# Black-Phoenix/CUDA-SfM

Measured on NVIDIA B200. Metric: RANSAC hyp*corr evals/s, higher is better.
Workload: dtype f32

## Files before the change

### cuda-sfm_b200/binding.py

```python
from __future__ import annotations

import ctypes as C
import os

HERE = os.path.dirname(os.path.abspath(__file__))


def lib_path() -> str:
    return os.path.join(HERE, "libsfmb200.so")


class SfmError(RuntimeError):
    def __init__(self, code: int, msg: str):
        super().__init__(f"sfmb200 error {code}: {msg}")
        self.code = code


_f = C.POINTER(C.c_float)
_i = C.POINTER(C.c_int32)
_vp = C.c_void_p

SIGNATURES = {
    "sfmb200_last_error": (C.c_char_p, []),
    "sfmb200_version": (C.c_int, []),
    "sfmb200_build_info": (C.c_char_p, []),
    "sfmb200_small_path_debug": (C.c_int, [_vp]),
    "sfmb200_create": (C.c_int, [_f, _f, C.c_int, C.c_int, C.c_int, C.POINTER(_vp)]),
    "sfmb200_destroy": (C.c_int, [_vp]),
    "sfmb200_set_option": (C.c_int, [_vp, C.c_int, C.c_int]),
    "sfmb200_set_stream": (C.c_int, [_vp, _vp]),
    "sfmb200_synchronize": (C.c_int, [_vp]),
    "sfmb200_set_points_sift": (C.c_int, [_vp, _vp, C.c_int]),
    "sfmb200_set_points_sift_filtered": (C.c_int, [_vp, _vp, C.c_int, C.c_float, C.c_float, _vp, C.POINTER(C.c_int32)]),
    "sfmb200_set_points_xy": (C.c_int, [_vp, _vp, C.c_int]),
    "sfmb200_set_points_xy_host": (C.c_int, [_vp, _vp, C.c_int]),
    "sfmb200_set_points_normalised": (C.c_int, [_vp, _vp, C.c_int]),
    "sfmb200_estimate_e": (C.c_int, [_vp, _vp, C.c_int, C.c_uint64, C.c_float]),
    "sfmb200_estimate_e_slice": (C.c_int, [_vp, _vp, C.c_int, C.c_int, C.c_int, C.c_uint64, C.c_float]),
    "sfmb200_copy_to_vbo_coloured": (C.c_int, [_vp, C.c_int, _vp, _vp, C.c_float, C.c_int, C.c_float, C.c_float]),
    "sfmb200_mg_handle_bytes": (C.c_int, []),
    "sfmb200_mg_init": (C.c_int, [_vp, C.c_int, C.c_int, _vp]),
    "sfmb200_mg_connect": (C.c_int, [_vp, _vp]),
    "sfmb200_estimate_e_mg": (C.c_int, [_vp, _vp, C.c_int, C.c_uint64, C.c_float]),
    "sfmb200_mg_status": (C.c_int, [_vp, _vp]),
    "sfmb200_mg_set_timeout_ms": (C.c_int, [_vp, C.c_int]),
    "sfmb200_mg_close": (C.c_int, [_vp]),
    "sfmb200_chain_views": (C.c_int, [_vp, _vp, _vp, _vp, _vp, _vp]),
    "sfmb200_bundle_adjust_global": (C.c_int, [_vp, _vp, _vp, C.c_int, _vp, _vp]),
    "sfmb200_bundle_adjust": (C.c_int, [_vp, C.c_int, C.c_int, _vp]),
    "sfmb200_estimate_e_adaptive": (C.c_int, [_vp, _vp, C.c_int, C.c_int, C.c_int, C.c_uint64, C.c_float, C.c_float, _vp]),
    "sfmb200_best_buffer": (C.c_int, [_vp, C.POINTER(_vp)]),
    "sfmb200_adopt_best": (C.c_int, [_vp, _vp, C.c_int, C.c_uint64]),
    "sfmb200_find_homography": (C.c_int, [_vp, C.c_int, C.c_uint64, C.c_float, _vp, _vp]),
    "sfmb200_refine_e": (C.c_int, [_vp, C.c_int]),
    "sfmb200_get_refit_iterations": (C.c_int, [_vp, _vp]),
    "sfmb200_pose_candidates": (C.c_int, [_vp]),
    "sfmb200_choose_pose": (C.c_int, [_vp]),
    "sfmb200_triangulate": (C.c_int, [_vp]),
    "sfmb200_run_host": (C.c_int, [_vp, _vp, C.c_int, C.c_int, C.c_uint64, C.c_float, _vp, _vp, _vp, _vp, _vp]),
    "sfmb200_run_device": (C.c_int, [_vp, _vp, C.c_int, C.c_int, C.c_uint64, C.c_float]),
    "sfmb200_copy_to_vbo": (C.c_int, [_vp, C.c_int, _vp, _vp]),
    "sfmb200_get_E": (C.c_int, [_vp, _vp]),
    "sfmb200_set_E": (C.c_int, [_vp, _vp]),
    "sfmb200_get_best": (C.c_int, [_vp, _vp, _vp]),
    "sfmb200_get_poses": (C.c_int, [_vp, _vp]),
    "sfmb200_get_pose_index": (C.c_int, [_vp, _vp]),
    "sfmb200_get_points": (C.c_int, [_vp, C.c_int, _vp]),
    "sfmb200_get_points_host": (C.c_int, [_vp, C.c_int, _vp]),
    "sfmb200_get_inlier_counts": (C.c_int, [_vp, C.c_int, _vp]),
    "sfmb200_get_E_candidates": (C.c_int, [_vp, C.c_int, _vp]),
    "sfmb200_get_X": (C.c_int, [_vp, C.c_int, C.c_int, _vp]),
    "sfmb200_get_inlier_mask": (C.c_int, [_vp, C.c_int, _vp]),
    "sfmb200_device_views": (C.c_int, [_vp, C.POINTER(_vp), C.POINTER(_vp), C.POINTER(_vp), C.POINTER(_vp), C.POINTER(C.c_int)]),
    "sfmb200_score_plan": (C.c_int, [_vp, _i]),
    "sfmb200_launch_count": (C.c_int64, [_vp]),
    "sfmb200_stage_times": (C.c_int, [_vp, C.c_int, _vp, C.POINTER(C.c_int)]),
    "sfmb200_fma_probe": (C.c_int, [C.c_int, C.c_int, C.POINTER(C.c_double), C.POINTER(C.c_float)]),
    "sfmb200_host_svd3": (None, [_f, _f, _f, _f]),
    "sfmb200_host_svd3_reference_orientation": (None, [_f, _f, _f, _f]),
    "sfmb200_host_solve_hypothesis": (None, [_f, _f]),
    "sfmb200_host_solve_hypothesis_projector": (None, [_f, _f]),
    "sfmb200_host_null4": (None, [_f, _f]),
    "sfmb200_host_null4_fast": (C.c_int, [_f, _f]),
    "sfmb200_host_dlt_null": (C.c_int, [_f, _f]),
    "sfmb200_host_dlt_null_power4": (None, [_f, _f]),
    "sfmb200_host_inv4": (C.c_int, [_f, _f]),
    "sfmb200_host_sample_indices": (None, [C.c_uint64, C.c_uint64, C.c_int, _i]),
    "sfmb200_host_sample_indices_disjoint": (None, [C.c_uint64, C.c_uint64, C.c_int, _i]),
    "sfmb200_la_mmul": (C.c_int, [_vp, _vp, _vp, C.c_int, C.c_int, C.c_int, _vp]),
    "sfmb200_la_mmul_batched": (C.c_int, [_vp, _vp, _vp, C.c_int, C.c_int, C.c_int, C.c_int, C.c_int, C.c_int, C.c_int, _vp]),
    "sfmb200_la_mmul_transpose_batched": (C.c_int, [_vp, _vp, _vp, C.c_int, C.c_int, C.c_int, C.c_int, C.c_int, C.c_int, C.c_int, _vp]),
    "sfmb200_la_invert": (C.c_int, [_vp, _vp, C.c_int, C.c_int, _vp]),
    "sfmb200_la_svd_batched": (C.c_int, [_vp, _vp, _vp, _vp, C.c_int, C.c_int, C.c_int, _vp]),
    "sfmb200_la_transpose_batched": (C.c_int, [_vp, _vp, C.c_int, C.c_int, C.c_int, _vp]),
    "sfmb200_la_vecnorm": (C.c_int, [_vp, _vp, C.c_int, C.c_int, C.c_float, C.c_float, _vp]),
    "sfmb200_la_elementwise": (C.c_int, [C.c_int, _vp, _vp, C.c_int, _vp]),
    "sfmb200_la_threshold_count": (C.c_int, [_vp, _vp, C.c_int, C.c_int, C.c_float, _vp]),
    "sfmb200_la_row_extraction": (C.c_int, [_vp, _vp, C.c_int, _vp]),
    "sfmb200_la_argmax_first": (C.c_int, [_vp, C.c_int, _i, _vp]),
    "sfmb200_la_copy_point": (C.c_int, [_vp, C.c_int, _vp, _vp, _vp]),
    "sfmb200_la_design_matrix": (C.c_int, [_vp, _vp, _vp, _vp, C.c_int, C.c_int, _vp]),
    "sfmb200_la_normalize_E": (C.c_int, [_vp, C.c_int, _vp]),
    "sfmb200_la_candidate_poses": (C.c_int, [_vp, _vp, _vp, _vp]),
    "sfmb200_la_triangulation_A": (C.c_int, [_vp, _vp, _vp, C.c_int, C.c_int, _vp, _vp, C.c_int, C.c_int, _vp]),
    "sfmb200_la_normalize_pt": (C.c_int, [_vp, _vp, C.c_int, _vp]),
    "sfmb200_la_copy_to_vbo": (C.c_int, [C.c_int, _vp, _vp, C.c_float, _vp]),
}


class Lib:

    def __init__(self, path: str | None = None):
        path = path or lib_path()
        if not os.path.exists(path):
            raise FileNotFoundError(
                f"{path} is missing: build it with `python cuda-sfm_b200/build.py` "
                "(there is no CPU fallback for the sfmb200 hot path)"
            )
        self.path = path
        self.cdll = C.CDLL(path)
        for name, (res, args) in SIGNATURES.items():
            fn = getattr(self.cdll, name)
            fn.restype = res
            fn.argtypes = args
            setattr(self, "_" + name, fn)

    def last_error(self) -> str:
        return self._sfmb200_last_error().decode()

    def call(self, name: str, *args):
        rc = getattr(self, "_" + name)(*args)
        if rc != 0:
            raise SfmError(rc, self.last_error())
        return rc

    def raw(self, name: str):
        return getattr(self, "_" + name)


_LIB: Lib | None = None


def load_library(path: str | None = None) -> Lib:
    global _LIB
    if _LIB is None or (path and path != _LIB.path):
        _LIB = Lib(path)
    return _LIB
```

### cuda-sfm_b200/csrc/api.cu

```cuda
#include <cuda_runtime.h>
#include <math.h>
#include <stdio.h>
#include <string.h>

#include <new>

#include "../../include/sfmb200.h"
#include "internal.cuh"
#include "sampson.cuh"

using namespace sfmb200;

static thread_local char g_err[512] = "";

static int fail(int code, const char* fmt, const char* detail = "") {
    snprintf(g_err, sizeof(g_err), fmt, detail);
    return code;
}
#define CK(call)                                                                     \
    do {                                                                             \
        cudaError_t e_ = (call);                                                     \
        if (e_ != cudaSuccess) return fail(SFMB200_ERR_CUDA, #call ": %s", cudaGetErrorString(e_)); \
    } while (0)
#define CKL()                                                                        \
    do {                                                                             \
        cudaError_t e_ = cudaGetLastError();                                         \
        if (e_ != cudaSuccess) return fail(SFMB200_ERR_CUDA, "kernel launch: %s", cudaGetErrorString(e_)); \
    } while (0)

struct sfmb200_handle {
    DeviceState s;
    RefitState refit;
    BAState ba;
    ChainState chain;
    void* chain_arena;
    GbaState gba;
    void* gba_arena;
    float* gba_stats;
    bool have_chain;
    void* staging_in;
    void* staging_out;
    void* ba_arena;
    MgPeers mg;
    void* mg_local;
    bool mg_connected;
    long long mg_calls;
    int* mg_failed_host;
    int* mg_failed_dev;
    int mg_clock_khz;
    long long mg_timeout_cycles;
    cudaStream_t stream;
    bool own_stream;
    cudaStream_t aux_stream;
    cudaEvent_t ev_fork;
    cudaEvent_t ev_chunk[16];
    int pipeline_chunks;
    int device;
    int sms;
    int compat;
    int score_variant;
    int tri_inliers_only;
    int hyp_solver;
    int small_path;
    long long small_evals;
    int model;
    int H;
    int h_begin;
    float thr;
    bool have_points, have_E, have_candidates, have_pose;
    ScorePlan plan;
    int64_t launches;
    int* filter_scratch;
    float* pack_header;
    float* pack_points;
    float* host_header;
    int* adapt;
    void* arena;
    int profile;
    int prof_cur;
    long long prof_total;
    cudaEvent_t (*prof_ev)[8];
    unsigned char* prof_mask;
};
static const int PROF_RING = 256;
static inline void prof_mark(sfmb200_handle* h, int k) {
    if (!h->profile) return;
    cudaEventRecord(h->prof_ev[h->prof_cur][k], h->stream);
    h->prof_mask[h->prof_cur] |= (unsigned char)(1u << k);
}
static inline void prof_next(sfmb200_handle* h) {
    if (!h->profile) return;
    h->prof_cur = (int)(h->prof_total % PROF_RING);
    h->prof_total++;
    h->prof_mask[h->prof_cur] = 0;
}

struct DeviceScope {
    int prev = -1;
    bool switched = false;
    cudaError_t err = cudaSuccess;
    explicit DeviceScope(const sfmb200_handle* h) {
        if (!h) return;
        err = cudaGetDevice(&prev);
        if (err == cudaSuccess && prev != h->device) {
            err = cudaSetDevice(h->device);
            switched = err == cudaSuccess;
        }
    }
    ~DeviceScope() {
        if (switched) cudaSetDevice(prev);
    }
};
#define ENTER(h)                                                                                          \
    DeviceScope scope_(h);                                                                                \
    if (scope_.err != cudaSuccess) return fail(SFMB200_ERR_CUDA, "cannot make the handle's device current: %s", cudaGetErrorString(scope_.err))

extern "C" {

const char* sfmb200_last_error(void) { return g_err; }
int sfmb200_version(void) { return 100; }

static size_t align_up(size_t v, size_t a) { return (v + a - 1) / a * a; }

int sfmb200_create(const float K[9], const float Kinv[9], int pairs, int max_points, int max_hyp, sfmb200_t** out) {
    if (!K || !Kinv || !out) return fail(SFMB200_ERR_ARG, "null argument%s");
    if (pairs < 1 || max_points < 8 || max_hyp < 1) return fail(SFMB200_ERR_ARG, "pairs >= 1, max_points >= 8, max_hypotheses >= 1 required%s");
    if (pairs > 65535) return fail(SFMB200_ERR_ARG, "at most 65535 pairs per handle (grid.y / grid.z limit)%s");
    int ndev = 0;
    if (cudaGetDeviceCount(&ndev) != cudaSuccess || ndev == 0) {
        cudaGetLastError();
        return fail(SFMB200_ERR_NODEVICE, "no CUDA device: sfmb200 has no CPU fallback%s");
    }
    sfmb200_handle* h = new (std::nothrow) sfmb200_handle();
    if (!h) return fail(SFMB200_ERR_ARG, "out of host memory%s");
    memset(h, 0, sizeof(*h));
    CK(cudaGetDevice(&h->device));
    CK(cudaDeviceGetAttribute(&h->sms, cudaDevAttrMultiProcessorCount, h->device));
    DeviceState& s = h->s;
    s.B = pairs;
    s.n_max = max_points;
    s.h_max = max_hyp;
    s.n = 0;
    s.n_stride = (int)align_up(max_points, SCORE_CHUNK);
    s.h_stride = (int)align_up(max_hyp, 1024);
    s.tiles_max = s.h_stride / SCORE_MIN_TILE;
    memcpy(s.K, K, sizeof(float) * 9);
    memcpy(s.Kinv, Kinv, sizeof(float) * 9);
    size_t B = pairs, off = 0;
    auto carve = [&](size_t bytes) { size_t o = off; off = align_up(off + bytes, 256); return o; };
    size_t o_corr = carve(B * s.n_stride * sizeof(float4));
    size_t o_cs = carve(B * s.n_stride * sizeof(float4));
    size_t o_ec = carve(B * 9 * (size_t)s.h_stride * sizeof(float));
    size_t o_cnt = carve(B * (size_t)s.h_stride * sizeof(int));
    size_t o_td = carve(B * (size_t)s.tiles_max * sizeof(int));
    size_t o_best = carve(B * sizeof(unsigned long long));
    size_t o_E = carve(B * 9 * sizeof(float));
    size_t o_bi = carve(B * sizeof(int));
    size_t o_bc = carve(B * sizeof(int));
    size_t o_P = carve(B * 64 * sizeof(float));
    size_t o_pi = carve(B * sizeof(int));
    size_t o_pts = carve(B * 4 * (size_t)s.n_stride * sizeof(float));
    size_t o_tc = carve(B * sizeof(int));
    size_t o_vote = carve(B * 8 * sizeof(int));
    size_t o_fs = carve(((size_t)max_points / 256 + 2) * sizeof(int));
    size_t o_ph = carve(B * 32 * sizeof(float));
    size_t o_ad = carve(4 * sizeof(int));
    const int refit_blocks = 64;
    size_t o_rc = carve(B * 9 * sizeof(float));
    size_t o_rT = carve(B * 8 * sizeof(float));
    size_t o_rf = carve(B * 4 * sizeof(int));
    size_t o_ri = carve(B * sizeof(int));
    size_t o_rm = carve(B * refit_blocks * 8 * sizeof(float));
    size_t o_rg = carve(B * refit_blocks * 45 * sizeof(float));
    cudaError_t e = cudaMalloc(&h->arena, off);
    if (e != cudaSuccess) {
        delete h;
        return fail(SFMB200_ERR_CUDA, "cudaMalloc(arena): %s", cudaGetErrorString(e));
    }
    char* base = (char*)h->arena;
    s.corr = (float4*)(base + o_corr);
    s.corr_s = (float4*)(base + o_cs);
    s.pt_scale = make_thr_scale(1e-6f).ik;
    s.px = nullptr;
    s.Ecand = (float*)(base + o_ec);
    s.counts = (int*)(base + o_cnt);
    s.tile_done = (int*)(base + o_td);
    s.best = (unsigned long long*)(base + o_best);
    s.E = (float*)(base + o_E);
    s.best_idx = (int*)(base + o_bi);
    s.best_count = (int*)(base + o_bc);
    s.P = (float*)(base + o_P);
    s.P_ind = (int*)(base + o_pi);
    s.points = (float*)(base + o_pts);
    s.tri_count = (int*)(base + o_tc);
    s.vote = (int*)(base + o_vote);
    h->filter_scratch = (int*)(base + o_fs);
    h->pack_header = (float*)(base + o_ph);
    h->pack_points = nullptr;
    h->adapt = (int*)(base + o_ad);
    h->ba.persistent = 1;
    h->refit.cand = (float*)(base + o_rc);
    h->refit.T = (float*)(base + o_rT);
    h->refit.flags = (int*)(base + o_rf);
    h->refit.iters_done = (int*)(base + o_ri);
    h->refit.mom_part = (float*)(base + o_rm);
    h->refit.gram_part = (float*)(base + o_rg);
    h->refit.max_blocks = refit_blocks;
    e = cudaMemset(h->arena, 0, off);
    if (e == cudaSuccess) e = cudaStreamCreateWithFlags(&h->stream, cudaStreamNonBlocking);
    if (e == cudaSuccess) e = cudaMallocHost((void**)&h->host_header, B * 32 * sizeof(float));
    if (e != cudaSuccess) {
        cudaFree(h->arena);
        delete h;
        return fail(SFMB200_ERR_CUDA, "create: %s", cudaGetErrorString(e));
    }
    h->own_stream = true;
    h->compat = 1;
    h->hyp_solver = 1;
    h->score_variant = -1;
    h->tri_inliers_only = 0;
    h->pipeline_chunks = -1;
    h->small_path = -1;
    h->small_evals = 2500000;
    *out = h;
    return SFMB200_OK;
}

int sfmb200_destroy(sfmb200_t* h) {
    ENTER(h);
    if (!h) return SFMB200_OK;
    cudaStreamSynchronize(h->stream);
    sfmb200_mg_close(h);
    if (h->aux_stream) {
        cudaStreamDestroy(h->aux_stream);
        cudaEventDestroy(h->ev_fork);
        for (int i = 0; i < 16; i++) cudaEventDestroy(h->ev_chunk[i]);
    }
    if (h->own_stream) cudaStreamDestroy(h->stream);
    if (h->host_header) cudaFreeHost(h->host_header);
    if (h->prof_ev) {
        for (int i = 0; i < PROF_RING; i++)
            for (int k = 0; k < 8; k++) cudaEventDestroy(h->prof_ev[i][k]);
        delete[] h->prof_ev;
        delete[] h->prof_mask;
    }
    cudaFree(h->arena);
    if (h->chain_arena) cudaFree(h->chain_arena);
    if (h->gba_arena) cudaFree(h->gba_arena);
    if (h->ba_arena) cudaFree(h->ba_arena);
    if (h->staging_in) cudaFree(h->staging_in);
    if (h->staging_out) cudaFree(h->staging_out);
    delete h;
    return SFMB200_OK;
}

int sfmb200_set_option(sfmb200_t* h, int option, int value) {
    ENTER(h);
    if (!h) return fail(SFMB200_ERR_ARG, "null handle%s");
    switch (option) {
        case SFMB200_OPT_COMPAT: h->compat = value ? 1 : 0; break;
        case SFMB200_OPT_SCORE_VARIANT:
            if (value < -1 || value >= score_num_variants()) return fail(SFMB200_ERR_ARG, "score variant out of range%s");
            h->score_variant = value;
            break;
        case SFMB200_OPT_TRI_INLIERS_ONLY: h->tri_inliers_only = value ? 1 : 0; break;
        case SFMB200_OPT_HYP_SOLVER:
            if (value < 0 || value > 1) return fail(SFMB200_ERR_ARG, "hypothesis solver must be 0 (Jacobi) or 1 (Cholesky projector)%s");
            h->hyp_solver = value;
            break;
        case SFMB200_OPT_BA_PERSISTENT: h->ba.persistent = value ? 1 : 0; break;
        case SFMB200_OPT_BATCH_PIPELINE:
            if (value < -1 || value > 16) return fail(SFMB200_ERR_ARG, "batch pipeline chunks must be -1 (auto), 0 / 1 (off) or 2..16%s");
            h->pipeline_chunks = value;
            break;
        case SFMB200_OPT_SAMPLER:
            if (value < 0 || value > 1) return fail(SFMB200_ERR_ARG, "sampler must be 0 (independent subsets) or 1 (disjoint permutation)%s");
            h->s.sampler = value;
            break;
        case SFMB200_OPT_SCORE_METRIC:
            if (value < 0 || value > 1) return fail(SFMB200_ERR_ARG, "score metric must be 0 (Sampson error) or 1 (symmetric epipolar distance)%s");
            h->s.metric = value;
            break;
        case SFMB200_OPT_SMALL_PATH:
            if (value < -1 || value > 1) return fail(SFMB200_ERR_ARG, "small path must be -1 (auto), 0 (never) or 1 (whenever eligible)%s");
            h->small_path = value;
            break;
        case SFMB200_OPT_SMALL_PATH_EVALS:
            if (value < 0) return fail(SFMB200_ERR_ARG, "evaluation limit must be >= 0%s");
            h->small_evals = value;
            break;
        case SFMB200_OPT_PROFILE:
            if (value && !h->prof_ev) {
                h->prof_ev = new cudaEvent_t[PROF_RING][8];
                h->prof_mask = new unsigned char[PROF_RING]();
                for (int i = 0; i < PROF_RING; i++)
                    for (int k = 0; k < 8; k++) CK(cudaEventCreate(&h->prof_ev[i][k]));
            }
            h->profile = value ? 1 : 0;
            h->prof_total = 0;
            h->prof_cur = 0;
            if (h->prof_mask) memset(h->prof_mask, 0, PROF_RING);
            break;
        default: return fail(SFMB200_ERR_ARG, "unknown option%s");
    }
    return SFMB200_OK;
}

int sfmb200_set_stream(sfmb200_t* h, void* stream) {
    ENTER(h);
    if (!h) return fail(SFMB200_ERR_ARG, "null handle%s");
    if (h->own_stream) {
        cudaStreamSynchronize(h->stream);
        cudaStreamDestroy(h->stream);
        h->own_stream = false;
    }
    h->stream = (cudaStream_t)stream;
    return SFMB200_OK;
}

int sfmb200_synchronize(sfmb200_t* h) {
    ENTER(h);
    if (!h) return fail(SFMB200_ERR_ARG, "null handle%s");
    CK(cudaStreamSynchronize(h->stream));
    return SFMB200_OK;
}

static int check_n(sfmb200_t* h, const void* p, int n) {
    if (!h || !p) return fail(SFMB200_ERR_ARG, "null argument%s");
    if (n < 8 || n > h->s.n_max) return fail(SFMB200_ERR_ARG, "n must be in [8, max_points]%s");
    return SFMB200_OK;
}

int sfmb200_set_points_sift(sfmb200_t* h, const void* d_sift, int n) {
    ENTER(h);
    int rc = check_n(h, d_sift, n);
    if (rc) return rc;
    if (h->s.B != 1) return fail(SFMB200_ERR_ARG, "SiftPoint ingest needs pairs == 1%s");
    h->s.n = n;
    launch_ingest_sift(h->s, d_sift, n, h->stream);
    CKL();
    h->launches++;
    h->have_points = true;
    h->have_chain = false;
    return SFMB200_OK;
}
int sfmb200_set_points_sift_filtered(sfmb200_t* h, const void* d_sift, int n, float min_score, float max_ambiguity,
                                     int32_t* d_kept_index, int32_t* h_kept) {
    ENTER(h);
    int rc = check_n(h, d_sift, n);
    if (rc) return rc;
    if (h->s.B != 1) return fail(SFMB200_ERR_ARG, "SiftPoint ingest needs pairs == 1%s");
    h->have_points = false;
    launch_ingest_sift_filtered(h->s, d_sift, n, min_score, max_ambiguity, h->filter_scratch, d_kept_index, h->stream);
    CKL();
    h->launches += 3;
    int kept = 0;
    int blocks = (n + 255) / 256;
    CK(cudaMemcpyAsync(&kept, h->filter_scratch + blocks, sizeof(int), cudaMemcpyDeviceToHost, h->stream));
    CK(cudaStreamSynchronize(h->stream));
    if (h_kept) *h_kept = kept;
    if (kept < 8) return fail(SFMB200_ERR_STATE, "fewer than 8 correspondences survive the match filter%s");
    h->s.n = kept;
    h->have_points = true;
    h->have_chain = false;
    return SFMB200_OK;
}
static int ingest_xy(sfmb200_t* h, const float* d_px, int n, float scale) {
    int rc = check_n(h, d_px, n);
    if (rc) return rc;
    h->s.n = n;
    if (scale > 0.0f) h->s.pt_scale = scale;
    prof_mark(h, 0);
    launch_ingest_xy(h->s, d_px, n, h->stream);
    prof_mark(h, 1);
    CKL();
    h->launches++;
    h->have_points = true;
    h->have_chain = false;
    return SFMB200_OK;
}
int sfmb200_set_points_xy(sfmb200_t* h, const float* d_px, int n) {
    ENTER(h);
    return ingest_xy(h, d_px, n, 0.0f);
}
static int ensure_staging(sfmb200_handle* h, bool in, bool out) {
    if (in && !h->staging_in) {
        CK(cudaMalloc(&h->staging_in, (size_t)h->s.B * h->s.n_stride * 4 * sizeof(float)));
        h->s.px = (float*)h->staging_in;
    }
    if (out && !h->staging_out) {
        CK(cudaMalloc(&h->staging_out, (size_t)h->s.B * 4 * (size_t)h->s.n_max * sizeof(float)));
        h->pack_points = (float*)h->staging_out;
    }
    return SFMB200_OK;
}

static int ingest_xy_host(sfmb200_t* h, const float* h_px, int n, float scale) {
    int rc = check_n(h, h_px, n);
    if (rc) return rc;
    if ((rc = ensure_staging(h, true, false))) return rc;
    CK(cudaMemcpyAsync(h->s.px, h_px, (size_t)h->s.B * n * 4 * sizeof(float), cudaMemcpyHostToDevice, h->stream));
    return ingest_xy(h, h->s.px, n, scale);
}
int sfmb200_set_points_xy_host(sfmb200_t* h, const float* h_px, int n) {
    ENTER(h);
    return ingest_xy_host(h, h_px, n, 0.0f);
}
int sfmb200_set_points_normalised(sfmb200_t* h, const float* d_x, int n) {
    ENTER(h);
    int rc = check_n(h, d_x, n);
    if (rc) return rc;
    h->s.n = n;
    launch_ingest_normalised(h->s, d_x, n, h->stream);
    CKL();
    h->launches++;
    h->have_points = true;
    h->have_chain = false;
    return SFMB200_OK;
}

static int ensure_scaled(sfmb200_handle* h, float scale) {
    if (h->s.pt_scale == scale) return SFMB200_OK;
    h->s.pt_scale = scale;
    launch_rescale_points(h->s, h->stream);
    CKL();
    h->launches++;
    return SFMB200_OK;
}

static void score_essential(sfmb200_handle* h, const DeviceState& s, int H, int h_offset, float thr) {
    if (s.metric == 0) launch_score(s, h->plan, H, h_offset, thr, h->stream);
    else launch_score_symmetric(s, h->plan, H, h_offset, thr, h->stream);
}
static ScorePlan plan_essential(const sfmb200_handle* h, int n, int H) {
    return h->s.metric == 0 ? make_score_plan(h->s.B, n, H, h->score_variant, h->sms) : make_score_plan_homography(h->s.B, n, H, h->sms);
}

constexpr int SMALL_PATH_MAX_PAIRS = 4;
static bool small_path_ok(const sfmb200_handle* h, int H, bool pose) {
    if (h->small_path == 0 || h->profile || h->hyp_solver != 1 || h->s.skip != nullptr || h->s.metric != 0) return false;
    if (h->score_variant >= 0 && h->small_path != 1) return false;
    if (pose && !h->compat) return false;
    if (H > small_path_max_hypotheses()) return false;
    if (h->small_path == 1) return true;
    if (h->s.B > SMALL_PATH_MAX_PAIRS) return false;
    return (long long)h->s.n * (long long)H <= h->small_evals;
}

int sfmb200_estimate_e_slice(sfmb200_t* h, const int32_t* d_idx, int H_total, int h_begin, int H, uint64_t seed,
                             float thr) {
    ENTER(h);
    if (!h) return fail(SFMB200_ERR_ARG, "null handle%s");
    if (!h->have_points) return fail(SFMB200_ERR_STATE, "estimate_e before set_points%s");
    if (H < 1 || H > h->s.h_max || h_begin < 0 || (long long)h_begin + H > (long long)H_total)
        return fail(SFMB200_ERR_ARG, "hypothesis slice out of range / above max_hypotheses%s");
    if (!(thr > 0.0f)) return fail(SFMB200_ERR_ARG, "threshold must be positive%s");
    if (!d_idx && h->s.sampler == 1 && 8ll * H_total > (long long)h->s.n)
        return fail(SFMB200_ERR_ARG, "the disjoint-permutation sampler needs 8 * H_total <= n (the reference uses H = N / 8)%s");
    h->H = H;
    h->h_begin = h_begin;
    h->thr = thr;
    if (int rc = ensure_scaled(h, make_thr_scale(thr).ik)) return rc;
    if (small_path_ok(h, H, false)) {
        CK(launch_small_path(h->s, nullptr, d_idx, (long long)H_total * 8, H, h_begin, seed, thr, h->compat, 0, SMALL_ESTIMATE, h->stream));
        memset(&h->plan, 0, sizeof(h->plan));
        h->plan.variant = -2;
        h->launches += 1;
    } else {
        h->plan = plan_essential(h, h->s.n, H);
        launch_hypgen(h->s, d_idx, (long long)H_total * 8, H, h_begin, seed, h->hyp_solver, h->stream);
        prof_mark(h, 2);
        CKL();
        score_essential(h, h->s, H, h_begin, thr);
        prof_mark(h, 3);
        CKL();
        launch_select(h->s, h_begin, h->stream);
        prof_mark(h, 4);
        CKL();
        h->launches += 3;
    }
    h->have_candidates = true;
    h->have_E = true;
    h->have_pose = false;
    h->have_chain = false;
    h->model = 0;
    return SFMB200_OK;
}

int sfmb200_find_homography(sfmb200_t* h, int loops, uint64_t seed, float thresh, float* h_H, int32_t* h_matches) {
    ENTER(h);
    if (!h) return fail(SFMB200_ERR_ARG, "null handle%s");
    if (!h->have_points) return fail(SFMB200_ERR_STATE, "find_homography before set_points%s");
    if (loops < 1 || loops > h->s.h_max) return fail(SFMB200_ERR_ARG, "loops out of range / above max_hypotheses%s");
    if (!(thresh > 0.0f)) return fail(SFMB200_ERR_ARG, "threshold must be positive%s");
    const float* Kc = h->s.K;
    const float f = Kc[0];
    const bool isotropic = f > 0.0f && fabsf(Kc[4] - f) <= 1e-6f * f && Kc[1] == 0.0f && Kc[3] == 0.0f && Kc[6] == 0.0f &&
                           Kc[7] == 0.0f && Kc[8] == 1.0f;
    if (!isotropic)
        return fail(SFMB200_ERR_ARG, "find_homography needs K = [f 0 cx; 0 f cy; 0 0 1] (square pixels, no skew): the pixel threshold is applied as thresh / f%s");
    const float thresh_n = thresh / f;
    const float thr2 = thresh_n * thresh_n;
    if (int rc = ensure_scaled(h, 1.0f)) return rc;
    h->H = loops;
    h->h_begin = 0;
    h->thr = thr2;
    h->plan = make_score_plan_homography(h->s.B, h->s.n, loops, h->sms);
    launch_hypgen(h->s, nullptr, (long long)loops * 8, loops, 0, seed, 2, h->stream);
    CKL();
    launch_score_homography(h->s, h->plan, loops, 0, thr2, h->stream);
    CKL();
    launch_select(h->s, 0, h->stream);
    CKL();
    h->launches += 3;
    h->have_candidates = true;
    h->have_E = false;
    h->have_pose = false;
    h->have_chain = false;
    h->model = 1;
    if (h_H) CK(cudaMemcpyAsync(h_H, h->s.E, (size_t)h->s.B * 9 * sizeof(float), cudaMemcpyDeviceToHost, h->stream));
    if (h_matches) CK(cudaMemcpyAsync(h_matches, h->s.best_count, (size_t)h->s.B * sizeof(int), cudaMemcpyDeviceToHost, h->stream));
    if (h_H || h_matches) CK(cudaStreamSynchronize(h->stream));
    if (h_H) {
        for (int b = 0; b < h->s.B; b++) {
            float* Hm = h_H + 9 * b;
            double T[9], R[9];
            for (int i = 0; i < 3; i++)
                for (int j = 0; j < 3; j++) {
                    double a = 0.0;
                    for (int k = 0; k < 3; k++) a += (double)Hm[3 * i + k] * (double)h->s.Kinv[3 * k + j];
                    T[3 * i + j] = a;
                }
            for (int i = 0; i < 3; i++)
                for (int j = 0; j < 3; j++) {
                    double a = 0.0;
                    for (int k = 0; k < 3; k++) a += (double)h->s.K[3 * i + k] * T[3 * k + j];
                    R[3 * i + j] = a;
                }
            const double inv = fabs(R[8]) > 1e-12 ? 1.0 / R[8] : 1.0;
            for (int i = 0; i < 9; i++) Hm[i] = (float)(R[i] * inv);
        }
    }
    return SFMB200_OK;
}
int sfmb200_estimate_e(sfmb200_t* h, const int32_t* d_idx, int H, uint64_t seed, float thr) {
    ENTER(h);
    return sfmb200_estimate_e_slice(h, d_idx, H, 0, H, seed, thr);
}

int sfmb200_estimate_e_adaptive(sfmb200_t* h, const int32_t* d_idx, int H_max, int first_round, int growth,
                                uint64_t seed, float thr, float confidence, int32_t* h_used) {
    ENTER(h);
    if (!h) return fail(SFMB200_ERR_ARG, "null handle%s");
    if (!h->have_points) return fail(SFMB200_ERR_STATE, "estimate_e before set_points%s");
    if (H_max < 1 || first_round < 1 || growth < 2) return fail(SFMB200_ERR_ARG, "H_max >= 1, first_round >= 1, growth >= 2 required%s");
    if (!(thr > 0.0f)) return fail(SFMB200_ERR_ARG, "threshold must be positive%s");
    if (!(confidence > 0.0f && confidence < 1.0f)) return fail(SFMB200_ERR_ARG, "confidence must be in (0, 1)%s");
    {
        long long lo = 0, hi = first_round;
        while (lo < H_max) {
            if (hi > H_max) hi = H_max;
            if (hi - lo > h->s.h_max) return fail(SFMB200_ERR_ARG, "a round exceeds max_hypotheses of the handle%s");
            lo = hi;
            hi *= growth;
        }
    }
    const double log1mp = log1p(-(double)confidence);
    if (int rc = ensure_scaled(h, make_thr_scale(thr).ik)) return rc;
    CK(cudaMemsetAsync(h->adapt, 0, 4 * sizeof(int), h->stream));
    DeviceState s = h->s;
    s.skip = h->adapt;
    long long lo = 0, hi = first_round;
    int rounds = 0;
    while (lo < H_max) {
        if (hi > H_max) hi = H_max;
        const int Hr = (int)(hi - lo);
        h->plan = plan_essential(h, s.n, Hr);
        launch_hypgen(s, d_idx, (long long)H_max * 8, Hr, (int)lo, seed, h->hyp_solver, h->stream, rounds > 0);
        CKL();
        score_essential(h, s, Hr, (int)lo, thr);
        CKL();
        launch_adaptive_decide(s, h->adapt, (int)lo, (int)hi, log1mp, hi >= H_max, h->stream);
        CKL();
        h->launches += 3;
        rounds++;
        h->H = Hr;
        h->h_begin = (int)lo;
        lo = hi;
        hi *= growth;
    }
    h->thr = thr;
    h->have_candidates = false;
    h->have_E = true;
    h->have_pose = false;
    h->have_chain = false;
    h->model = 0;
    if (h_used) {
        CK(cudaMemcpyAsync(h_used, h->adapt + 1, sizeof(int), cudaMemcpyDeviceToHost, h->stream));
        CK(cudaStreamSynchronize(h->stream));
    }
    return SFMB200_OK;
}

struct MgBlob {
    cudaIpcMemHandle_t ipc;
    unsigned char uuid[16];
};
int sfmb200_mg_handle_bytes(void) { return (int)sizeof(MgBlob); }

int sfmb200_mg_init(sfmb200_t* h, int rank, int world, void* h_handle_out) {
    ENTER(h);
    if (!h || !h_handle_out) return fail(SFMB200_ERR_ARG, "null argument%s");
    if (world < 1 || world > MG_MAX_WORLD || rank < 0 || rank >= world) return fail(SFMB200_ERR_ARG, "bad rank / world (at most 16 ranks)%s");
    if (h->mg_local) return fail(SFMB200_ERR_STATE, "mg_init called twice%s");
    const size_t bytes = mg_buffer_bytes(h->s.B, world);
    CK(cudaMalloc(&h->mg_local, bytes));
    CK(cudaMemset(h->mg_local, 0, bytes));
    CK(cudaHostAlloc((void**)&h->mg_failed_host, sizeof(int), cudaHostAllocMapped));
    *h->mg_failed_host = 0;
    CK(cudaHostGetDevicePointer((void**)&h->mg_failed_dev, h->mg_failed_host, 0));
    MgBlob blob;
    memset(&blob, 0, sizeof(blob));
    CK(cudaIpcGetMemHandle(&blob.ipc, h->mg_local));
    cudaDeviceProp prop;
    CK(cudaGetDeviceProperties(&prop, h->device));
    memcpy(blob.uuid, prop.uuid.bytes, 16);
    memcpy(h_handle_out, &blob, sizeof(blob));
    memset(&h->mg, 0, sizeof(h->mg));
    h->mg.rank = rank;
    h->mg.world = world;
    h->mg.base[rank] = (unsigned long long*)h->mg_local;
    h->mg_connected = false;
    h->mg_calls = 0;
    int clock_khz = 0;
    cudaDeviceGetAttribute(&clock_khz, cudaDevAttrClockRate, h->device);
    h->mg_clock_khz = clock_khz > 0 ? clock_khz : 1900000;
    h->mg_timeout_cycles = 2000LL * h->mg_clock_khz;
    return SFMB200_OK;
}

int sfmb200_mg_set_timeout_ms(sfmb200_t* h, int ms) {
    ENTER(h);
    if (!h || ms < 1) return fail(SFMB200_ERR_ARG, "timeout must be >= 1 ms%s");
    if (!h->mg_local) return fail(SFMB200_ERR_STATE, "mg_set_timeout_ms before mg_init%s");
    h->mg_timeout_cycles = (long long)ms * h->mg_clock_khz;
    return SFMB200_OK;
}

int sfmb200_mg_connect(sfmb200_t* h, const void* h_handles) {
    ENTER(h);
    if (!h || !h_handles) return fail(SFMB200_ERR_ARG, "null argument%s");
    if (!h->mg_local) return fail(SFMB200_ERR_STATE, "mg_connect before mg_init%s");
    if (h->mg_connected) return fail(SFMB200_ERR_STATE, "mg_connect called twice%s");
    const MgBlob* all = (const MgBlob*)h_handles;
    int ndev = 0;
    CK(cudaGetDeviceCount(&ndev));
    for (int r = 0; r < h->mg.world; r++) {
        if (r == h->mg.rank) continue;
        int peer_dev = -1;
        for (int d = 0; d < ndev && peer_dev < 0; d++) {
            cudaDeviceProp prop;
            CK(cudaGetDeviceProperties(&prop, d));
            if (memcmp(prop.uuid.bytes, all[r].uuid, 16) == 0) peer_dev = d;
        }
        if (peer_dev < 0) return fail(SFMB200_ERR_ARG, "mg_connect: a peer's device is not visible to this process%s");
        if (peer_dev != h->device) {
            int native = 0;
            CK(cudaDeviceGetP2PAttribute(&native, cudaDevP2PAttrNativeAtomicSupported, h->device, peer_dev));
            if (!native) return fail(SFMB200_ERR_STATE, "mg_connect: no native P2P atomics between this device and a peer (not NVLink-connected)%s");
        }
        void* p = nullptr;
        CK(cudaIpcOpenMemHandle(&p, all[r].ipc, cudaIpcMemLazyEnablePeerAccess));
        h->mg.base[r] = (unsigned long long*)p;
    }
    h->mg_connected = true;
    return SFMB200_OK;
}

int sfmb200_mg_close(sfmb200_t* h) {
    ENTER(h);
    if (!h) return SFMB200_OK;
    if (h->mg_local) {
        cudaStreamSynchronize(h->stream);
        for (int r = 0; r < h->mg.world; r++)
            if (r != h->mg.rank && h->mg.base[r]) cudaIpcCloseMemHandle(h->mg.base[r]);
        cudaFree(h->mg_local);
        cudaFreeHost(h->mg_failed_host);
        h->mg_local = nullptr;
        h->mg_failed_host = nullptr;
        h->mg_failed_dev = nullptr;
        h->mg_connected = false;
        memset(&h->mg, 0, sizeof(h->mg));
    }
    return SFMB200_OK;
}

int sfmb200_estimate_e_mg(sfmb200_t* h, const int32_t* d_idx, int H_total, uint64_t seed, float thr) {
    ENTER(h);
    if (!h) return fail(SFMB200_ERR_ARG, "null handle%s");
    if (!h->mg_connected) return fail(SFMB200_ERR_STATE, "estimate_e_mg before mg_init / mg_connect%s");
    if (*(volatile int*)h->mg_failed_host != 0) {
        h->have_E = false;
        h->have_candidates = false;
        return fail(SFMB200_ERR_STATE, "the peer exchange timed out earlier (a rank is lost or late): sfmb200_mg_close + mg_init + mg_connect on every rank%s");
    }
    const int world = h->mg.world, rank = h->mg.rank;
    if (H_total < world) return fail(SFMB200_ERR_ARG, "fewer hypotheses than ranks%s");
    const long long base = H_total / world, rem = H_total % world;
    const long long lo = rank * base + (rank < rem ? rank : rem), cnt = base + (rank < rem ? 1 : 0);
    int rc = sfmb200_estimate_e_slice(h, d_idx, H_total, (int)lo, (int)cnt, seed, thr);
    if (rc) return rc;
    launch_mg_exchange(h->s, h->mg, h->mg_calls, H_total, h->mg_timeout_cycles, h->mg_failed_dev, h->stream);
    CKL();
    h->mg_calls++;
    h->launches += 2;
    h->have_candidates = false;
    return SFMB200_OK;
}

int sfmb200_mg_status(sfmb200_t* h, int32_t* h_timeouts) {
    ENTER(h);
    if (!h || !h_timeouts) return fail(SFMB200_ERR_ARG, "null argument%s");
    *h_timeouts = 0;
    if (!h->mg_failed_host) return SFMB200_OK;
    CK(cudaStreamSynchronize(h->stream));
    *h_timeouts = *(volatile int*)h->mg_failed_host;
    if (*h_timeouts != 0) h->have_E = false;
    return SFMB200_OK;
}

int sfmb200_best_buffer(sfmb200_t* h, uint64_t** d_best) {
    ENTER(h);
    if (!h || !d_best) return fail(SFMB200_ERR_ARG, "null argument%s");
    *d_best = (uint64_t*)h->s.best;
    return SFMB200_OK;
}
int sfmb200_adopt_best(sfmb200_t* h, const int32_t* d_idx, int H_total, uint64_t seed) {
    ENTER(h);
    if (!h) return fail(SFMB200_ERR_ARG, "null handle%s");
    if (!h->have_points) return fail(SFMB200_ERR_STATE, "adopt_best before set_points%s");
    if (h->model != 0 || !(h->thr > 0.0f))
        return fail(SFMB200_ERR_STATE, "adopt_best follows an essential-matrix estimate (estimate_e / estimate_e_slice) on this handle%s");
    launch_regen_best(h->s, d_idx, (long long)H_total * 8, seed, h->hyp_solver, h->stream);
    CKL();
    h->launches++;
    h->have_E = true;
    h->have_pose = false;
    h->have_chain = false;
    h->model = 0;
    return SFMB200_OK;
}

int sfmb200_refine_e(sfmb200_t* h, int iterations) {
    ENTER(h);
    if (!h) return fail(SFMB200_ERR_ARG, "null handle%s");
    if (iterations < 0 || iterations > 64) return fail(SFMB200_ERR_ARG, "iterations must be in [0, 64]%s");
    if (!h->have_E || !h->have_points) return fail(SFMB200_ERR_STATE, "refine_e before an essential matrix exists%s");
    if (iterations == 0) return SFMB200_OK;
    h->launches += launch_refit(h->s, h->refit, h->thr > 0 ? h->thr : 1e-6f, iterations, h->stream);
    CKL();
    h->have_pose = false;
    h->have_chain = false;
    return SFMB200_OK;
}
static int ensure_ba_arena(sfmb200_handle* h) {
    if (h->ba_arena) return SFMB200_OK;
    const DeviceState& s = h->s;
    const size_t B = s.B;
    int ba_blocks = (592 + s.B - 1) / s.B;
    ba_blocks = ba_blocks < 2 ? 2 : (ba_blocks > 296 ? 296 : ba_blocks);
    size_t off = 0;
    auto carve = [&](size_t bytes) { size_t o = off; off = align_up(off + bytes, 256); return o; };
    size_t o_bp = carve(B * 2 * 3 * (size_t)s.n_stride * sizeof(float));
    size_t o_ba = carve(B * (size_t)s.n_stride);
    size_t o_bc2 = carve(B * 24 * sizeof(float));
    size_t o_bd = carve(B * 6 * sizeof(double));
    size_t o_bi2 = carve(B * 8 * sizeof(int));
    size_t o_bf = carve(B * 8 * sizeof(float));
    size_t o_bpart = carve(B * ba_blocks * 34 * sizeof(double));
    size_t o_bpart2 = carve(B * ba_blocks * 2 * sizeof(double));
    size_t o_bs = carve(B * 8 * sizeof(float));
    size_t o_bcand = carve(B * 32 * sizeof(float));
    size_t o_bbase = carve(B * sizeof(int));
    CK(cudaMalloc(&h->ba_arena, off));
    CK(cudaMemsetAsync(h->ba_arena, 0, off, h->stream));
    char* base = (char*)h->ba_arena;
    h->ba.pts = (float*)(base + o_bp);
    h->ba.active = (unsigned char*)(base + o_ba);
    h->ba.cam = (float*)(base + o_bc2);
    h->ba.dc = (double*)(base + o_bd);
    h->ba.ctl_i = (int*)(base + o_bi2);
    h->ba.ctl_f = (float*)(base + o_bf);
    h->ba.part = (double*)(base + o_bpart);
    h->ba.part2 = (double*)(base + o_bpart2);
    h->ba.stats = (float*)(base + o_bs);
    h->ba.cand = (float*)(base + o_bcand);
    h->ba.base_count = (int*)(base + o_bbase);
    h->ba.max_blocks = ba_blocks;
    return SFMB200_OK;
}

int sfmb200_bundle_adjust(sfmb200_t* h, int outer_rounds, int iterations, float* h_stats) {
    ENTER(h);
    if (!h) return fail(SFMB200_ERR_ARG, "null handle%s");
    if (outer_rounds < 1 || outer_rounds > 64 || iterations < 1 || iterations > 256)
        return fail(SFMB200_ERR_ARG, "outer_rounds in [1, 64] and iterations in [1, 256] required%s");
    if (!h->have_points || !h->have_E || !h->have_pose || h->model != 0)
        return fail(SFMB200_ERR_STATE, "bundle_adjust needs an essential matrix and a chosen pose%s");
    const float thr = h->thr > 0 ? h->thr : 1e-6f;
    if (int rc = ensure_ba_arena(h)) return rc;
    for (int r = 0; r < outer_rounds; r++) {
        h->launches += launch_bundle_adjust(h->s, h->ba, thr, iterations, 1e-3f, h->tri_inliers_only, r == 0, h->ba.stats, h->stream);
        CKL();
    }
    if (h_stats) {
        CK(cudaMemcpyAsync(h_stats, h->ba.stats, (size_t)h->s.B * 8 * sizeof(float), cudaMemcpyDeviceToHost, h->stream));
        CK(cudaStreamSynchronize(h->stream));
    }
    return SFMB200_OK;
}

int sfmb200_chain_views(sfmb200_t* h, float* d_cloud, int32_t* d_count, float* h_cameras, float* h_scales, int32_t* h_used) {
    ENTER(h);
    if (!h) return fail(SFMB200_ERR_ARG, "null handle%s");
    if (h->s.B > 256) return fail(SFMB200_ERR_ARG, "chain_views handles at most 256 pairs (257 views)%s");
    if (!h->have_points || !h->have_E || !h->have_pose || h->model != 0)
        return fail(SFMB200_ERR_STATE, "chain_views needs an essential matrix, a chosen pose and triangulated points per pair%s");
    const size_t B = h->s.B;
    if (!h->chain_arena) {
        size_t off = 0;
        auto carve = [&](size_t bytes) { size_t o = off; off = align_up(off + bytes, 256); return o; };
        size_t o_h = carve(B * 2048 * sizeof(int)), o_m = carve(B * sizeof(int)), o_u = carve(B * sizeof(int));
        size_t o_s = carve(B * sizeof(unsigned long long)), o_c = carve(B * sizeof(int)), o_sc = carve(B * sizeof(float));
        size_t o_cs = carve(B * sizeof(float)), o_cam = carve((B + 1) * 12 * sizeof(float));
        CK(cudaMalloc(&h->chain_arena, off));
        char* base = (char*)h->chain_arena;
        h->chain.hist = (int*)(base + o_h);
        h->chain.median_bin = (int*)(base + o_m);
        h->chain.used = (int*)(base + o_u);
        h->chain.bin_sum = (unsigned long long*)(base + o_s);
        h->chain.bin_cnt = (int*)(base + o_c);
        h->chain.scales = (float*)(base + o_sc);
        h->chain.cum_scales = (float*)(base + o_cs);
        h->chain.cameras = (float*)(base + o_cam);
        CK(cudaMemsetAsync(h->chain_arena, 0, off, h->stream));
    }
    h->launches += launch_chain(h->s, h->chain, h->thr > 0 ? h->thr : 1e-6f, d_cloud, d_count, h->stream);
    CKL();
    if (h_cameras) CK(cudaMemcpyAsync(h_cameras, h->chain.cameras, (B + 1) * 12 * sizeof(float), cudaMemcpyDeviceToHost, h->stream));
    if (h_scales) CK(cudaMemcpyAsync(h_scales, h->chain.scales, B * sizeof(float), cudaMemcpyDeviceToHost, h->stream));
    if (h_used) CK(cudaMemcpyAsync(h_used, h->chain.used, B * sizeof(int), cudaMemcpyDeviceToHost, h->stream));
    if (h_cameras || h_scales || h_used) CK(cudaStreamSynchronize(h->stream));
    h->have_chain = true;
    return SFMB200_OK;
}

int sfmb200_bundle_adjust_global(sfmb200_t* h, float* d_cloud, const int32_t* d_count, int iterations, float* h_cameras,
                                 float* h_stats) {
    ENTER(h);
    if (!h || !d_cloud || !d_count) return fail(SFMB200_ERR_ARG, "null argument%s");
    if (iterations < 1 || iterations > 1000) return fail(SFMB200_ERR_ARG, "iterations must be in [1, 1000]%s");
    if (h->s.B > GBA_MAX_PAIRS) return fail(SFMB200_ERR_ARG, "bundle_adjust_global handles at most 16 pairs (17 views)%s");
    if (!h->have_chain || !h->chain_arena || !h->have_points || !h->have_E || !h->have_pose || h->model != 0)
        return fail(SFMB200_ERR_STATE, "bundle_adjust_global follows chain_views (cloud and count from that call)%s");
    const DeviceState& s = h->s;
    if (!h->gba_arena) {
        const size_t V = s.B + 1, n = s.n_max;
        const int nb = 148;
        size_t off = 0;
        auto carve = [&](size_t bytes) { size_t o = off; off = align_up(off + bytes, 256); return o; };
        size_t o_cam = carve(2 * V * 12 * sizeof(float)), o_pts = carve(2 * 3 * n * sizeof(float)), o_obs = carve(n * sizeof(unsigned int));
        size_t o_lin = carve(n * 9 * sizeof(float)), o_part = carve(gba_part_doubles(s.B, nb) * sizeof(double));
        size_t o_p2 = carve((size_t)nb * 2 * sizeof(double)), o_dc = carve(6 * (size_t)s.B * sizeof(double));
        size_t o_ci = carve(8 * sizeof(int)), o_cf = carve(8 * sizeof(float)), o_st = carve(8 * sizeof(float));
        CK(cudaMalloc(&h->gba_arena, off));
        CK(cudaMemsetAsync(h->gba_arena, 0, off, h->stream));
        char* base = (char*)h->gba_arena;
        h->gba.cam = (float*)(base + o_cam);
        h->gba.pts = (float*)(base + o_pts);
        h->gba.obs = (unsigned int*)(base + o_obs);
        h->gba.lin = (float*)(base + o_lin);
        h->gba.part = (double*)(base + o_part);
        h->gba.part2 = (double*)(base + o_p2);
        h->gba.dc = (double*)(base + o_dc);
        h->gba.ctl_i = (int*)(base + o_ci);
        h->gba.ctl_f = (float*)(base + o_cf);
        h->gba.nb = nb;
        h->gba_stats = (float*)(base + o_st);
    }
    float* d_stats = h->gba_stats;
    h->launches += launch_global_ba(h->s, h->chain, h->gba, h->thr > 0 ? h->thr : 1e-6f, iterations, d_cloud, d_count, d_stats, h->stream);
    CKL();
    const size_t B = h->s.B;
    if (h_cameras) CK(cudaMemcpyAsync(h_cameras, h->chain.cameras, (B + 1) * 12 * sizeof(float), cudaMemcpyDeviceToHost, h->stream));
    if (h_stats) CK(cudaMemcpyAsync(h_stats, d_stats, 8 * sizeof(float), cudaMemcpyDeviceToHost, h->stream));
    if (h_cameras || h_stats) CK(cudaStreamSynchronize(h->stream));
    return SFMB200_OK;
}

int sfmb200_get_refit_iterations(sfmb200_t* h, int32_t* h_iters) {
    ENTER(h);
    if (!h || !h_iters) return fail(SFMB200_ERR_ARG, "null argument%s");
    CK(cudaMemcpyAsync(h_iters, h->refit.iters_done, (size_t)h->s.B * sizeof(int), cudaMemcpyDeviceToHost, h->stream));
    CK(cudaStreamSynchronize(h->stream));
    return SFMB200_OK;
}

int sfmb200_pose_candidates(sfmb200_t* h) {
    ENTER(h);
    if (!h) return fail(SFMB200_ERR_ARG, "null handle%s");
    if (!h->have_E) return fail(SFMB200_ERR_STATE, "pose_candidates before an essential matrix exists%s");
    launch_pose_candidates(h->s, h->compat, h->stream);
    prof_mark(h, 5);
    CKL();
    h->launches++;
    h->have_pose = true;
    return SFMB200_OK;
}
int sfmb200_choose_pose(sfmb200_t* h) {
    ENTER(h);
    if (!h) return fail(SFMB200_ERR_ARG, "null handle%s");
    if (!h->have_pose || !h->have_points) return fail(SFMB200_ERR_STATE, "choose_pose before pose_candidates%s");
    launch_choose_pose(h->s, h->compat, h->thr > 0 ? h->thr : 1e-6f, h->stream);
    prof_mark(h, 6);
    CKL();
    h->launches++;
    return SFMB200_OK;
}
int sfmb200_triangulate(sfmb200_t* h) {
    ENTER(h);
    if (!h) return fail(SFMB200_ERR_ARG, "null handle%s");
    if (!h->have_pose || !h->have_points) return fail(SFMB200_ERR_STATE, "triangulate before pose_candidates%s");
    launch_triangulate(h->s, h->tri_inliers_only, h->thr > 0 ? h->thr : 1e-6f, h->stream);
    prof_mark(h, 7);
    CKL();
    h->launches++;
    return SFMB200_OK;
}

static int run_stages(sfmb200_t* h, int H, uint64_t seed, float thr) {
    if (!h->have_points) return fail(SFMB200_ERR_STATE, "run before set_points%s");
    if (H < 1 || H > h->s.h_max) return fail(SFMB200_ERR_ARG, "H out of range / above max_hypotheses%s");
    if (!(thr > 0.0f)) return fail(SFMB200_ERR_ARG, "threshold must be positive%s");
    h->H = H;
    h->h_begin = 0;
    h->thr = thr;
    if (int rc = ensure_scaled(h, make_thr_scale(thr).ik)) return rc;
    h->plan = plan_essential(h, h->s.n, H);
    int chunks = h->pipeline_chunks;
    if (chunks < 0) chunks = 1;
    if (chunks > h->s.B) chunks = h->s.B;
    if (chunks >= 2) {
        if (!h->aux_stream) {
            CK(cudaStreamCreateWithFlags(&h->aux_stream, cudaStreamNonBlocking));
            CK(cudaEventCreateWithFlags(&h->ev_fork, cudaEventDisableTiming));
            for (int i = 0; i < 16; i++) CK(cudaEventCreateWithFlags(&h->ev_chunk[i], cudaEventDisableTiming));
        }
        CK(cudaEventRecord(h->ev_fork, h->stream));
        CK(cudaStreamWaitEvent(h->aux_stream, h->ev_fork, 0));
        const int per = (h->s.B + chunks - 1) / chunks;
        int used = 0;
        for (int c = 0, b0 = 0; b0 < h->s.B; c++, b0 += per, used++) {
            const DeviceState v = sub_batch(h->s, b0, b0 + per <= h->s.B ? per : h->s.B - b0);
            launch_hypgen(v, nullptr, (long long)H * 8, H, 0, seed, h->hyp_solver, h->aux_stream);
            CKL();
            CK(cudaEventRecord(h->ev_chunk[c], h->aux_stream));
        }
        for (int c = 0, b0 = 0; b0 < h->s.B; c++, b0 += per) {
            const DeviceState v = sub_batch(h->s, b0, b0 + per <= h->s.B ? per : h->s.B - b0);
            CK(cudaStreamWaitEvent(h->stream, h->ev_chunk[c], 0));
            ScorePlan keep = h->plan;
            h->plan = h->s.metric == 0 ? make_score_plan(v.B, v.n, H, h->score_variant, h->sms) : make_score_plan_homography(v.B, v.n, H, h->sms);
            score_essential(h, v, H, 0, thr);
            CKL();
            h->plan = keep;
        }
        h->launches += 2 * used - 2;
    } else {
        launch_hypgen(h->s, nullptr, (long long)H * 8, H, 0, seed, h->hyp_solver, h->stream);
        prof_mark(h, 2);
        CKL();
        score_essential(h, h->s, H, 0, thr);
        prof_mark(h, 3);
        CKL();
    }
    launch_select_pose_choose(h->s, 0, h->compat, h->stream);
    prof_mark(h, 4);
    prof_mark(h, 5);
    CKL();
    h->launches += 3;
    if (!h->compat) {
        launch_choose_pose(h->s, 0, thr, h->stream);
        CKL();
        h->launches++;
    }
    prof_mark(h, 6);
    h->have_candidates = h->have_E = h->have_pose = true;
    h->have_chain = false;
    h->model = 0;
    return sfmb200_triangulate(h);
}

static int run_small(sfmb200_t* h, const float* d_px, int n, int H, uint64_t seed, float thr) {
    if (!d_px || n < 8 || n > h->s.n_max || H < 1 || H > h->s.h_max) return 0;
    const int n_before = h->s.n;
    h->s.n = n;
    const bool ok = small_path_ok(h, H, true);
    h->s.n = n_before;
    if (!ok) return 0;
    h->s.n = n;
    h->s.pt_scale = make_thr_scale(thr).ik;
    cudaError_t e = launch_small_path(h->s, d_px, nullptr, (long long)H * 8, H, 0, seed, thr, h->compat, h->tri_inliers_only,
                                      SMALL_INGEST | SMALL_ESTIMATE | SMALL_POSE | SMALL_TRI, h->stream);
    if (e != cudaSuccess) return fail(SFMB200_ERR_CUDA, "fused small-problem launch: %s", cudaGetErrorString(e));
    h->H = H;
    h->h_begin = 0;
    h->thr = thr;
    h->model = 0;
    memset(&h->plan, 0, sizeof(h->plan));
    h->plan.variant = -2;
    h->launches += 1;
    h->have_points = h->have_candidates = h->have_E = h->have_pose = true;
    h->have_chain = false;
    return 1;
}

int sfmb200_run_device(sfmb200_t* h, const float* d_px, int n, int H, uint64_t seed, float thr) {
    ENTER(h);
    if (!h) return fail(SFMB200_ERR_ARG, "null handle%s");
    if (!(thr > 0.0f)) return fail(SFMB200_ERR_ARG, "threshold must be positive%s");
    prof_next(h);
    if (int rc = run_small(h, d_px, n, H, seed, thr)) return rc < 0 ? rc : SFMB200_OK;
    int rc = ingest_xy(h, d_px, n, make_thr_scale(thr).ik);
    if (rc) return rc;
    return run_stages(h, H, seed, thr);
}

__global__ void pack_results_kernel(DeviceState s, float* header, float* points, int want_points) {
    const int b = blockIdx.y;
    if (blockIdx.x == 0 && threadIdx.x < 32) {
        const int t = threadIdx.x;
        float v = 0.0f;
        if (t < 9) v = s.E[(size_t)b * 9 + t];
        else if (t < 25) v = s.P[(size_t)b * 64 + 16 * s.P_ind[b] + (t - 9)];
        else if (t == 25) v = __int_as_float(s.P_ind[b]);
        else if (t == 26) v = __int_as_float(s.best_count[b]);
        else if (t == 27) v = __int_as_float(s.best_idx[b]);
        header[(size_t)b * 32 + t] = v;
    }
    if (!want_points) return;
    const int i = blockIdx.x * blockDim.x + threadIdx.x;
    if (i >= s.n) return;
    const float* in = s.points + (size_t)b * 4 * s.n_stride;
    float* out = points + (size_t)b * 4 * s.n;
#pragma unroll
    for (int r = 0; r < 4; r++) out[(size_t)r * s.n + i] = in[(size_t)r * s.n_stride + i];
}

static void* pinned_alias(const void* host) {
    if (!host) return nullptr;
    cudaPointerAttributes a;
    if (cudaPointerGetAttributes(&a, host) != cudaSuccess) {
        cudaGetLastError();
        return nullptr;
    }
    return a.type == cudaMemoryTypeHost ? a.devicePointer : nullptr;
}

int sfmb200_run_host(sfmb200_t* h, const float* h_px, int n, int H, uint64_t seed, float thr, float* h_E, float* h_P,
                     int32_t* h_pose_index, int32_t* h_inliers, float* h_points) {
    ENTER(h);
    if (!h) return fail(SFMB200_ERR_ARG, "null handle%s");
    if (!(thr > 0.0f)) return fail(SFMB200_ERR_ARG, "threshold must be positive%s");
    prof_next(h);
    const float scale = make_thr_scale(thr).ik;
    const size_t zero_copy_limit = 4u << 20;
    const size_t in_bytes = (size_t)h->s.B * (size_t)(n > 0 ? n : 0) * 4 * sizeof(float);
    const float* px_alias = in_bytes <= zero_copy_limit ? (const float*)pinned_alias(h_px) : nullptr;
    int rc = 0;
    const bool small_shape = h_px && n >= 8 && n <= h->s.n_max && H >= 1 && H <= h->s.h_max;
    if (px_alias) {
        rc = run_small(h, px_alias, n, H, seed, thr);
    } else if (small_shape) {
        if ((rc = ensure_staging(h, true, false))) return rc;
        CK(cudaMemcpyAsync(h->s.px, h_px, (size_t)h->s.B * n * 4 * sizeof(float), cudaMemcpyHostToDevice, h->stream));
        rc = run_small(h, h->s.px, n, H, seed, thr);
        if (rc == 0) {
            if ((rc = ingest_xy(h, h->s.px, n, scale))) return rc;
            if ((rc = run_stages(h, H, seed, thr))) return rc;
            rc = 1;
        }
    }
    if (rc < 0) return rc;
    if (rc == 0) {
        rc = px_alias ? ingest_xy(h, px_alias, n, scale) : ingest_xy_host(h, h_px, n, scale);
        if (rc) return rc;
        if ((rc = run_stages(h, H, seed, thr))) return rc;
    }
    DeviceState& s = h->s;
    const size_t B = s.B;
    float* pts_alias = B * 4 * (size_t)s.n * sizeof(float) <= zero_copy_limit ? (float*)pinned_alias(h_points) : nullptr;
    if (h_points && !pts_alias && (rc = ensure_staging(h, false, true))) return rc;
    dim3 grid(h_points ? (s.n + 255) / 256 : 1, (unsigned)B);
    pack_results_kernel<<<grid, 256, 0, h->stream>>>(s, h->host_header, pts_alias ? pts_alias : h->pack_points, h_points ? 1 : 0);
    CKL();
    h->launches++;
    if (h_points && !pts_alias)
        CK(cudaMemcpyAsync(h_points, h->pack_points, B * 4 * (size_t)s.n * sizeof(float), cudaMemcpyDeviceToHost, h->stream));
    CK(cudaStreamSynchronize(h->stream));
    for (size_t b = 0; b < B; b++) {
        const float* hd = h->host_header + b * 32;
        if (h_E) memcpy(h_E + b * 9, hd, 9 * sizeof(float));
        if (h_P) memcpy(h_P + b * 16, hd + 9, 16 * sizeof(float));
        if (h_pose_index) memcpy(h_pose_index + b, hd + 25, sizeof(int32_t));
        if (h_inliers) memcpy(h_inliers + b, hd + 26, sizeof(int32_t));
    }
    return SFMB200_OK;
}

int sfmb200_copy_to_vbo(sfmb200_t* h, int pair, float* d_pos, float* d_col) {
    ENTER(h);
    if (!h || pair < 0 || pair >= h->s.B) return fail(SFMB200_ERR_ARG, "bad handle / pair%s");
    launch_vbo(h->s, pair, d_pos, d_col, 1.0f, h->stream);
    CKL();
    h->launches++;
    CK(cudaStreamSynchronize(h->stream));
    return SFMB200_OK;
}

int sfmb200_copy_to_vbo_coloured(sfmb200_t* h, int pair, float* d_pos, float* d_col, float scale, int mode, float z_near, float z_far) {
    ENTER(h);
    if (!h || pair < 0 || pair >= h->s.B) return fail(SFMB200_ERR_ARG, "bad handle / pair%s");
    if (mode < 0 || mode > 2) return fail(SFMB200_ERR_ARG, "colour mode must be 0 (ones), 1 (inlier / outlier) or 2 (depth ramp)%s");
    if (mode == 1 && (!h->have_E || h->model != 0)) return fail(SFMB200_ERR_STATE, "inlier colouring needs an essential matrix%s");
    launch_vbo_colour(h->s, pair, d_pos, d_col, scale, mode, h->thr > 0 ? h->thr : 1e-6f, z_near, z_far, h->stream);
    CKL();
    h->launches++;
    CK(cudaStreamSynchronize(h->stream));
    return SFMB200_OK;
}

int sfmb200_get_E(sfmb200_t* h, float* h_E) {
    ENTER(h);
    if (!h || !h_E) return fail(SFMB200_ERR_ARG, "null argument%s");
    CK(cudaMemcpyAsync(h_E, h->s.E, (size_t)h->s.B * 9 * sizeof(float), cudaMemcpyDeviceToHost, h->stream));
    CK(cudaStreamSynchronize(h->stream));
    return SFMB200_OK;
}
int sfmb200_set_E(sfmb200_t* h, const float* h_E) {
    ENTER(h);
    if (!h || !h_E) return fail(SFMB200_ERR_ARG, "null argument%s");
    CK(cudaMemcpyAsync(h->s.E, h_E, (size_t)h->s.B * 9 * sizeof(float), cudaMemcpyHostToDevice, h->stream));
    CK(cudaStreamSynchronize(h->stream));
    h->have_E = true;
    h->have_pose = false;
    h->have_chain = false;
    h->model = 0;
    if (!(h->thr > 0)) h->thr = 1e-6f;
    return SFMB200_OK;
}
int sfmb200_get_best(sfmb200_t* h, int32_t* h_index, int32_t* h_count) {
    ENTER(h);
    if (!h) return fail(SFMB200_ERR_ARG, "null argument%s");
    if (h_index) CK(cudaMemcpyAsync(h_index, h->s.best_idx, (size_t)h->s.B * sizeof(int), cudaMemcpyDeviceToHost, h->stream));
    if (h_count) CK(cudaMemcpyAsync(h_count, h->s.best_count, (size_t)h->s.B * sizeof(int), cudaMemcpyDeviceToHost, h->stream));
    CK(cudaStreamSynchronize(h->stream));
    return SFMB200_OK;
}
int sfmb200_get_poses(sfmb200_t* h, float* h_P) {
    ENTER(h);
    if (!h || !h_P) return fail(SFMB200_ERR_ARG, "null argument%s");
    CK(cudaMemcpyAsync(h_P, h->s.P, (size_t)h->s.B * 64 * sizeof(float), cudaMemcpyDeviceToHost, h->stream));
    CK(cudaStreamSynchronize(h->stream));
    return SFMB200_OK;
}
int sfmb200_get_pose_index(sfmb200_t* h, int32_t* h_ind) {
    ENTER(h);
    if (!h || !h_ind) return fail(SFMB200_ERR_ARG, "null argument%s");
    CK(cudaMemcpyAsync(h_ind, h->s.P_ind, (size_t)h->s.B * sizeof(int), cudaMemcpyDeviceToHost, h->stream));
    CK(cudaStreamSynchronize(h->stream));
    return SFMB200_OK;
}
static int check_pair(sfmb200_t* h, int pair, const void* p) {
    if (!h || !p) return fail(SFMB200_ERR_ARG, "null argument%s");
    if (pair < 0 || pair >= h->s.B) return fail(SFMB200_ERR_ARG, "pair out of range%s");
    return SFMB200_OK;
}
int sfmb200_get_points(sfmb200_t* h, int pair, float* d_points) {
    ENTER(h);
    int rc = check_pair(h, pair, d_points);
    if (rc) return rc;
    const DeviceState& s = h->s;
    CK(cudaMemcpy2DAsync(d_points, (size_t)s.n * sizeof(float), s.points + (size_t)pair * 4 * s.n_stride,
                         (size_t)s.n_stride * sizeof(float), (size_t)s.n * sizeof(float), 4, cudaMemcpyDeviceToDevice,
                         h->stream));
    return SFMB200_OK;
}
int sfmb200_get_points_host(sfmb200_t* h, int pair, float* h_points) {
    ENTER(h);
    int rc = check_pair(h, pair, h_points);
    if (rc) return rc;
    const DeviceState& s = h->s;
    CK(cudaMemcpy2DAsync(h_points, (size_t)s.n * sizeof(float), s.points + (size_t)pair * 4 * s.n_stride,
                         (size_t)s.n_stride * sizeof(float), (size_t)s.n * sizeof(float), 4, cudaMemcpyDeviceToHost,
                         h->stream));
    CK(cudaStreamSynchronize(h->stream));
    return SFMB200_OK;
}
int sfmb200_get_inlier_counts(sfmb200_t* h, int pair, int32_t* d_counts) {
    ENTER(h);
    int rc = check_pair(h, pair, d_counts);
    if (rc) return rc;
    if (!h->have_candidates) return fail(SFMB200_ERR_STATE, "no estimate yet%s");
    CK(cudaMemcpyAsync(d_counts, h->s.counts + (size_t)pair * h->s.h_stride, (size_t)h->H * sizeof(int),
                       cudaMemcpyDeviceToDevice, h->stream));
    return SFMB200_OK;
}
int sfmb200_get_E_candidates(sfmb200_t* h, int pair, float* d_E) {
    ENTER(h);
    int rc = check_pair(h, pair, d_E);
    if (rc) return rc;
    if (!h->have_candidates) return fail(SFMB200_ERR_STATE, "no estimate yet%s");
    launch_export_ecand(h->s, pair, h->H, d_E, h->stream);
    CKL();
    h->launches++;
    return SFMB200_OK;
}
int sfmb200_get_X(sfmb200_t* h, int pair, int image, float* d_X) {
    ENTER(h);
    int rc = check_pair(h, pair, d_X);
    if (rc) return rc;
    if (image < 0 || image > 1) return fail(SFMB200_ERR_ARG, "image must be 0 or 1%s");
    if (!h->have_points) return fail(SFMB200_ERR_STATE, "no points yet%s");
    launch_export_X(h->s, pair, image, d_X, h->stream);
    CKL();
    h->launches++;
    return SFMB200_OK;
}
int sfmb200_get_inlier_mask(sfmb200_t* h, int pair, uint8_t* d_mask) {
    ENTER(h);
    int rc = check_pair(h, pair, d_mask);
    if (rc) return rc;
    if (!(h->have_E || h->model == 1) || !h->have_points) return fail(SFMB200_ERR_STATE, "no model yet%s");
    launch_inlier_mask(h->s, pair, h->thr > 0 ? h->thr : 1e-6f, h->model, d_mask, h->stream);
    CKL();
    h->launches++;
    return SFMB200_OK;
}
int sfmb200_device_views(sfmb200_t* h, float** d_E, float** d_P, int32_t** d_pose_index, float** d_points,
                         int* point_stride) {
    ENTER(h);
    if (!h) return fail(SFMB200_ERR_ARG, "null handle%s");
    if (d_E) *d_E = h->s.E;
    if (d_P) *d_P = h->s.P;
    if (d_pose_index) *d_pose_index = h->s.P_ind;
    if (d_points) *d_points = h->s.points;
    if (point_stride) *point_stride = h->s.n_stride;
    return SFMB200_OK;
}
int sfmb200_score_plan(sfmb200_t* h, int32_t out[4]) {
    ENTER(h);
    if (!h || !out) return fail(SFMB200_ERR_ARG, "null argument%s");
    out[0] = h->plan.variant;
    out[1] = h->plan.tiles;
    out[2] = h->plan.ctas;
    out[3] = h->plan.hyp_per_cta;
    return SFMB200_OK;
}
int64_t sfmb200_launch_count(sfmb200_t* h) { return h ? h->launches : 0; }

int sfmb200_stage_times(sfmb200_t* h, int max_sets, float* ms, int* sets) {
    ENTER(h);
    if (!h || !ms || !sets) return fail(SFMB200_ERR_ARG, "null argument%s");
    *sets = 0;
    if (!h->prof_ev) return fail(SFMB200_ERR_STATE, "profiling was never enabled%s");
    CK(cudaStreamSynchronize(h->stream));
    long long have = h->prof_total < PROF_RING ? h->prof_total : PROF_RING;
    long long first = h->prof_total - have;
    for (long long t = first; t < h->prof_total && *sets < max_sets; t++) {
        int i = (int)(t % PROF_RING);
        if (h->prof_mask[i] != 0xFF) continue;
        for (int k = 0; k < 7; k++) CK(cudaEventElapsedTime(&ms[(size_t)(*sets) * 7 + k], h->prof_ev[i][k], h->prof_ev[i][k + 1]));
        (*sets)++;
    }
    return SFMB200_OK;
}

int sfmb200_small_path_debug(int64_t* d_stamps) {
    small_path_set_debug((long long*)d_stamps);
    return SFMB200_OK;
}

int sfmb200_fma_probe(int mode, int iters, double* fmas, float* ms) {
    if (!fmas || !ms || iters < 1 || mode < 0 || mode > 4) return fail(SFMB200_ERR_ARG, "bad argument%s");
    float* sink = nullptr;
    cudaEvent_t e0, e1;
    CK(cudaMalloc(&sink, 256));
    CK(cudaEventCreate(&e0));
    CK(cudaEventCreate(&e1));
    launch_fma_probe(mode, 4, 0, sink);
    CK(cudaEventRecord(e0, 0));
    *fmas = launch_fma_probe(mode, iters, 0, sink);
    CK(cudaEventRecord(e1, 0));
    CK(cudaEventSynchronize(e1));
    CKL();
    CK(cudaEventElapsedTime(ms, e0, e1));
    cudaEventDestroy(e0);
    cudaEventDestroy(e1);
    cudaFree(sink);
    return SFMB200_OK;
}

}
```

### cuda-sfm_b200/csrc/internal.cuh

```cuda
#pragma once
#include <cuda_runtime.h>
#include <stdint.h>

namespace sfmb200 {

struct ScorePlan {
    int variant;
    int hyp_per_cta;
    int tiles;
    int n_units;
    long long total_units;
    int ctas;
};

#ifndef SFMB200_SCORE_CHUNK
#define SFMB200_SCORE_CHUNK 512
#endif
constexpr int SCORE_CHUNK = SFMB200_SCORE_CHUNK;
constexpr int SCORE_GRAIN = 64;
constexpr int SCORE_MIN_TILE = 256;

struct DeviceState {
    int B;
    int pair0;
    int n_max;
    int h_max;
    int n;
    int n_stride;
    int h_stride;
    int tiles_max;
    float Kinv[9];
    float K[9];

    float pt_scale;
    float4* corr;
    float4* corr_s;
    float* px;
    float* Ecand;
    int* counts;
    int* tile_done;
    unsigned long long* best;
    float* E;
    int* best_idx;
    int* best_count;
    float* P;
    int* P_ind;
    float* points;
    int* tri_count;
    int* vote;
    int sampler;
    int metric;
    const int* skip;
};

inline DeviceState sub_batch(const DeviceState& s, int b0, int nb) {
    DeviceState v = s;
    const size_t b = (size_t)b0;
    v.B = nb;
    v.pair0 = s.pair0 + b0;
    v.corr += b * s.n_stride;
    v.corr_s += b * s.n_stride;
    v.Ecand += b * 9 * s.h_stride;
    v.counts += b * s.h_stride;
    v.tile_done += b * s.tiles_max;
    v.best += b;
    v.E += b * 9;
    v.best_idx += b;
    v.best_count += b;
    v.P += b * 64;
    v.P_ind += b;
    v.points += b * 4 * s.n_stride;
    v.tri_count += b;
    v.vote += b * 8;
    return v;
}

struct RefitState {
    float* cand;
    float* T;
    int* flags;
    int* iters_done;
    float* mom_part;
    float* gram_part;
    int max_blocks;
};
int launch_refit(const DeviceState& s, const RefitState& r, float thr, int iterations, cudaStream_t st);

struct BAState {
    float* pts;
    unsigned char* active;
    float* cam;
    double* dc;
    int* ctl_i;
    float* ctl_f;
    double* part;
    double* part2;
    int persistent;
    float* stats;
    int* base_count;
    float* cand;
    int max_blocks;
};
constexpr int MG_MAX_WORLD = 16;
struct MgPeers {
    unsigned long long* base[MG_MAX_WORLD];
    int rank, world;
};
void launch_mg_exchange(const DeviceState& s, const MgPeers& peers, long long call, int H_total, long long timeout_cycles,
                        int* d_failed, cudaStream_t st);
size_t mg_buffer_bytes(int B, int world);

struct ChainState {
    int* hist;
    int* median_bin;
    int* used;
    unsigned long long* bin_sum;
    int* bin_cnt;
    float* scales;
    float* cum_scales;
    float* cameras;
};
int launch_chain(const DeviceState& s, const ChainState& c, float thr, float* d_cloud, int* d_count, cudaStream_t st);

struct GbaState {
    float* cam;
    float* pts;
    unsigned int* obs;
    float* lin;
    double* part;
    double* part2;
    double* dc;
    int* ctl_i;
    float* ctl_f;
    int nb;
};
constexpr int GBA_MAX_PAIRS = 16;
size_t gba_part_doubles(int pairs, int nb);
int launch_global_ba(const DeviceState& s, const ChainState& c, const GbaState& g, float thr, int iterations, float* d_cloud,
                     const int* d_count, float* d_stats, cudaStream_t st);

int launch_bundle_adjust(const DeviceState& s, const BAState& ba, float thr, int iterations, float lambda0,
                         int tri_inliers_only, int first_round, float* d_stats, cudaStream_t st);

void launch_ingest_sift(const DeviceState& s, const void* d_sift, int n, cudaStream_t st);
void launch_ingest_sift_filtered(const DeviceState& s, const void* d_sift, int n, float min_score, float max_ambiguity,
                                 int* d_scratch, int* d_kept_index, cudaStream_t st);
void launch_ingest_xy(const DeviceState& s, const float* d_px, int n, cudaStream_t st);
void launch_ingest_normalised(const DeviceState& s, const float* d_x, int n, cudaStream_t st);
void launch_rescale_points(const DeviceState& s, cudaStream_t st);
void launch_hypgen(const DeviceState& s, const int32_t* d_idx, long long idx_pair_stride, int H, int h_offset,
                   unsigned long long seed, int solver, cudaStream_t st, int keep_best = 0);
void launch_adaptive_decide(const DeviceState& s, int* d_adapt, int round_begin, int done_after, double log1mp, int last,
                            cudaStream_t st);
ScorePlan make_score_plan(int B, int n, int H, int variant_override, int sms);
int score_num_variants();
void launch_score(const DeviceState& s, const ScorePlan& plan, int H, int h_offset, float thr, cudaStream_t st);
void launch_score_homography(const DeviceState& s, ScorePlan& plan, int H, int h_offset, float thr2, cudaStream_t st);
void launch_score_symmetric(const DeviceState& s, ScorePlan& plan, int H, int h_offset, float thr, cudaStream_t st);
ScorePlan make_score_plan_homography(int B, int n, int H, int sms);
void launch_select(const DeviceState& s, int h_offset, cudaStream_t st);
void launch_regen_best(const DeviceState& s, const int32_t* d_idx, long long idx_pair_stride,
                       unsigned long long seed, int solver, cudaStream_t st);
void launch_pose_candidates(const DeviceState& s, int compat, cudaStream_t st);
void launch_select_pose_choose(const DeviceState& s, int h_offset, int compat, cudaStream_t st);
void launch_choose_pose(const DeviceState& s, int compat, float thr, cudaStream_t st);
void launch_triangulate(const DeviceState& s, int inliers_only, float thr, cudaStream_t st);
void launch_vbo(const DeviceState& s, int pair, float* d_pos, float* d_col, float scale, cudaStream_t st);
void launch_vbo_colour(const DeviceState& s, int pair, float* d_pos, float* d_col, float scale, int mode, float thr, float z_near,
                       float z_far, cudaStream_t st);
void launch_export_ecand(const DeviceState& s, int pair, int H, float* d_out_Hx9, cudaStream_t st);
void launch_export_X(const DeviceState& s, int pair, int image, float* d_out_3xN, cudaStream_t st);
void launch_inlier_mask(const DeviceState& s, int pair, float thr, int model, unsigned char* d_mask, cudaStream_t st);

enum { SMALL_INGEST = 1, SMALL_ESTIMATE = 2, SMALL_POSE = 4, SMALL_TRI = 8 };
int small_path_max_hypotheses();
void small_path_set_debug(long long* d_stamps);
cudaError_t launch_small_path(const DeviceState& s, const float* d_px, const int32_t* d_idx, long long idx_pair_stride, int H,
                              int h_offset, unsigned long long seed, float thr, int compat, int inliers_only, int mask,
                              cudaStream_t st);

#ifdef SFMB200_PDL
__device__ __forceinline__ void pdl_wait() { asm volatile("griddepcontrol.wait;" ::: "memory"); }
__device__ __forceinline__ void pdl_trigger() { asm volatile("griddepcontrol.launch_dependents;" ::: "memory"); }
template <typename... KArgs, typename... Args>
inline void launch_dep(void (*kernel)(KArgs...), dim3 grid, dim3 block, size_t smem, cudaStream_t st, Args... args) {
    cudaLaunchConfig_t cfg = {};
    cfg.gridDim = grid;
    cfg.blockDim = block;
    cfg.dynamicSmemBytes = smem;
    cfg.stream = st;
    cudaLaunchAttribute attr[1];
    attr[0].id = cudaLaunchAttributeProgrammaticStreamSerialization;
    attr[0].val.programmaticStreamSerializationAllowed = 1;
    cfg.attrs = attr;
    cfg.numAttrs = 1;
    cudaLaunchKernelEx(&cfg, kernel, KArgs(args)...);
}
#else
__device__ __forceinline__ void pdl_wait() {}
__device__ __forceinline__ void pdl_trigger() {}
template <typename... KArgs, typename... Args>
inline void launch_dep(void (*kernel)(KArgs...), dim3 grid, dim3 block, size_t smem, cudaStream_t st, Args... args) {
    kernel<<<grid, block, smem, st>>>(KArgs(args)...);
}
#endif

double launch_fma_probe(int mode, int iters, cudaStream_t st, float* d_sink);

}
```

### cuda-sfm_b200/csrc/score.cu

```cuda
#include <math.h>

#include <mutex>

#include "internal.cuh"
#include "sampson.cuh"

#ifndef SFMB200_SCORE_UNROLL
#define SFMB200_SCORE_UNROLL 2
#endif

namespace sfmb200 {

constexpr int kScoreUnroll = SFMB200_SCORE_UNROLL;

__device__ __forceinline__ uint32_t smem_u32(const void* p) { return (uint32_t)__cvta_generic_to_shared(p); }

__device__ __forceinline__ void mbar_init(uint64_t* bar, int count) {
    asm volatile("mbarrier.init.shared::cta.b64 [%0], %1;" ::"r"(smem_u32(bar)), "r"(count));
}
__device__ __forceinline__ void mbar_expect_tx(uint64_t* bar, uint32_t bytes) {
    asm volatile("mbarrier.arrive.expect_tx.shared::cta.b64 _, [%0], %1;" ::"r"(smem_u32(bar)), "r"(bytes) : "memory");
}
__device__ __forceinline__ void mbar_wait(uint64_t* bar, uint32_t parity) {
    uint32_t done;
    do {
        asm volatile(
            "{\n"
            ".reg .pred p;\n"
            "mbarrier.try_wait.parity.shared::cta.b64 p, [%1], %2;\n"
            "selp.u32 %0, 1, 0, p;\n"
            "}\n"
            : "=r"(done)
            : "r"(smem_u32(bar)), "r"(parity)
            : "memory");
    } while (!done);
}
__device__ __forceinline__ void tma_load_1d(void* dst, const void* src, uint32_t bytes, uint64_t* bar) {
    asm volatile("cp.async.bulk.shared::cluster.global.mbarrier::complete_tx::bytes [%0], [%1], %2, [%3];" ::"r"(
                     smem_u32(dst)),
                 "l"(src), "r"(bytes), "r"(smem_u32(bar))
                 : "memory");
}

__device__ __forceinline__ unsigned long long warp_max_u64(unsigned long long v) {
#pragma unroll
    for (int o = 16; o > 0; o >>= 1) {
        unsigned long long w = __shfl_xor_sync(0xFFFFFFFFu, v, o);
        v = w > v ? w : v;
    }
    return v;
}

struct ChunkWalk {
    long long u, end;
    int n_units, n, T;
    int b, t, p0, cnt;
    int seg_p0, seg_pts;
    int left;
    bool seg_first, seg_last;
    __device__ __forceinline__ void init(long long u0, long long u1, int n_units_, int n_, int T_) {
        u = u0; end = u1; n_units = n_units_; n = n_; T = T_;
        left = 0; cnt = 0; p0 = 0;
    }
    __device__ __forceinline__ bool next() {
        if (left == 0) {
            if (u >= end) return false;
            long long bt = u / n_units;
            int pu = (int)(u - bt * n_units);
            long long seg_units = end - u;
            if (seg_units > n_units - pu) seg_units = n_units - pu;
            b = (int)(bt / T);
            t = (int)(bt - (long long)b * T);
            seg_p0 = pu * SCORE_GRAIN;
            int p1 = (pu + (int)seg_units) * SCORE_GRAIN;
            if (p1 > n) p1 = n;
            seg_pts = p1 - seg_p0;
            left = seg_pts;
            u += seg_units;
            p0 = seg_p0;
            seg_first = true;
        } else {
            p0 += cnt;
            seg_first = false;
        }
        cnt = left < SCORE_CHUNK ? left : SCORE_CHUNK;
        left -= cnt;
        seg_last = (left == 0);
        return true;
    }
};

template <int HPT, int THREADS>
__device__ __forceinline__ void segment_epilogue(const DeviceState& s, int b, int t, int H, int h_offset,
                                                 const unsigned int* cnt, bool full, int inc, int total,
                                                 unsigned long long* red, int* s_last) {
    constexpr int HPC = HPT * THREADS;
    const int tid = threadIdx.x;
    int* counts = s.counts + (size_t)b * s.h_stride;
    unsigned long long key = 0ull;
    bool do_argmax;
    if (full) {
#pragma unroll
        for (int j = 0; j < HPT; j++) {
            int h = t * HPC + j * THREADS + tid;
            if (h < H) {
                counts[h] = (int)cnt[j];
                unsigned long long kk = ((unsigned long long)cnt[j] << 32) |
                                        (unsigned long long)(0xFFFFFFFFu - (unsigned)(h_offset + h));
                key = kk > key ? kk : key;
            }
        }
        do_argmax = true;
    } else {
#pragma unroll
        for (int j = 0; j < HPT; j++) {
            int h = t * HPC + j * THREADS + tid;
            if (h < H && cnt[j] != 0u) atomicAdd(&counts[h], (int)cnt[j]);
        }
        __threadfence();
        __syncthreads();
        if (tid == 0) {
            int before = atomicAdd(&s.tile_done[(size_t)b * s.tiles_max + t], inc);
            *s_last = (before + inc == total);
        }
        __syncthreads();
        do_argmax = *s_last != 0;
        if (do_argmax) {
            __threadfence();
#pragma unroll
            for (int j = 0; j < HPT; j++) {
                int h = t * HPC + j * THREADS + tid;
                if (h < H) {
                    unsigned int total = (unsigned int)__ldcg(&counts[h]);
                    unsigned long long kk = ((unsigned long long)total << 32) |
                                            (unsigned long long)(0xFFFFFFFFu - (unsigned)(h_offset + h));
                    key = kk > key ? kk : key;
                }
            }
        }
    }
    if (do_argmax) {
        key = warp_max_u64(key);
        if ((tid & 31) == 0) red[tid >> 5] = key;
        __syncthreads();
        if (tid < 32) {
            unsigned long long v = tid < THREADS / 32 ? red[tid] : 0ull;
            v = warp_max_u64(v);
            if (tid == 0 && v != 0ull) atomicMax(&s.best[b], v);
        }
        __syncthreads();
    }
}

struct ChunkDesc {
    int b, t;
    int cnt_flags;
    int seg_pts;
};

template <int HPT, bool PACKED, int THREADS, int MINB, int MODEL>
__global__ void __launch_bounds__(THREADS, MINB)
score_kernel(DeviceState s, int H, int h_offset, int T, long long total_units, int n_units, float thr) {
    constexpr int HPC = HPT * THREADS;
    __shared__ __align__(128) float4 buf[2][SCORE_CHUNK];
    __shared__ __align__(8) uint64_t full[2];
    __shared__ __align__(16) ChunkDesc desc[2];
    __shared__ ChunkWalk walk;
    __shared__ unsigned long long red[THREADS / 32];
    __shared__ int s_last;

    pdl_wait();
    pdl_trigger();
    if (s.skip != nullptr && *s.skip != 0) return;
    const int tid = threadIdx.x;
    if (tid == 0) {
        mbar_init(&full[0], 1);
        mbar_init(&full[1], 1);
        asm volatile("fence.mbarrier_init.release.cluster;" ::: "memory");
        ChunkWalk w;
        w.init(total_units * blockIdx.x / gridDim.x, total_units * (blockIdx.x + 1) / gridDim.x, n_units, s.n, T);
        walk = w;
    }
    __syncthreads();

    auto produce = [&](int stage) {
        ChunkWalk w = walk;
        bool more = w.next();
        walk = w;
        ChunkDesc d;
        d.b = w.b; d.t = w.t; d.seg_pts = w.seg_pts;
        d.cnt_flags = more ? (w.cnt | (w.seg_first ? (1 << 30) : 0) | (w.seg_last ? (1 << 31) : 0)) : 0;
        desc[stage] = d;
        if (more) {
            const float4* src = s.corr_s + (size_t)w.b * s.n_stride + w.p0;
            uint32_t bytes = (uint32_t)w.cnt * 16u;
            mbar_expect_tx(&full[stage], bytes);
            tma_load_1d(&buf[stage][0], src, bytes, &full[stage]);
        } else {
            mbar_expect_tx(&full[stage], 0);
        }
    };
    if (tid == 0) produce(0);

    float e[PACKED ? 1 : HPT][9];
    float2 e2[PACKED ? HPT / 2 : 1][9];
    unsigned int cnt[HPT];
    const float nthr = -thr;
    const float2 nthr2 = make_float2(nthr, nthr);
    const ThrScale ts = make_thr_scale(thr);
    (void)e; (void)e2; (void)nthr2; (void)ts;

    for (int k = 0;; k++) {
        if (tid == 0) produce((k + 1) & 1);
        mbar_wait(&full[k & 1], (k >> 1) & 1);
        const ChunkDesc d = desc[k & 1];
        if (d.cnt_flags == 0) break;
        const int n_here = d.cnt_flags & 0x3FFFFFFF;
        if (d.cnt_flags & (1 << 30)) {
            const float* Eb = s.Ecand + (size_t)d.b * 9 * s.h_stride;
#pragma unroll
            for (int j = 0; j < HPT; j++) {
                int h = d.t * HPC + j * THREADS + tid;
                bool valid = h < H;
#pragma unroll
                for (int q = 0; q < 9; q++) {
                    float v = valid ? __ldg(Eb + (size_t)q * s.h_stride + h) : 0.0f;
                    if (MODEL != 1 && q != 8) v *= thr_scale_factor(ts, q);
                    if constexpr (PACKED) {
                        if (j & 1) e2[j / 2][q].y = v; else e2[j / 2][q].x = v;
                    } else {
                        e[j][q] = v;
                    }
                }
                cnt[j] = 0u;
            }
        }
        const float4* pb = buf[k & 1];
        if constexpr (PACKED) {
#pragma unroll kScoreUnroll
            for (int i = 0; i < n_here; i++) {
                const float4 p = pb[i];
                const float2 x1 = make_float2(p.x, p.x), y1 = make_float2(p.y, p.y);
                const float2 x2 = make_float2(p.z, p.z), y2 = make_float2(p.w, p.w);
#pragma unroll
                for (int j = 0; j < HPT / 2; j++) {
                    float2 dd = model_d2<MODEL>(e2[j], x1, y1, x2, y2, nthr2);
                    cnt[2 * j] += __float_as_uint(dd.x) >> 31;
                    cnt[2 * j + 1] += __float_as_uint(dd.y) >> 31;
                }
            }
        } else {
#pragma unroll 4
            for (int i = 0; i < n_here; i++) {
                float4 p = pb[i];
#pragma unroll
                for (int j = 0; j < HPT; j++) {
                    float dd = model_d<MODEL>(e[j], p.x, p.y, p.z, p.w, nthr);
                    cnt[j] += __float_as_uint(dd) >> 31;
                }
            }
        }
        __syncthreads();
        if (d.cnt_flags >= 0) continue;

        segment_epilogue<HPT, THREADS>(s, d.b, d.t, H, h_offset, cnt, d.seg_pts == s.n, d.seg_pts, s.n, red, &s_last);
    }
}

constexpr int CONST_PTS = 4000;
__constant__ float4 c_pts[CONST_PTS];

template <int HPT, int THREADS, int MINB, int MODEL>
__global__ void __launch_bounds__(THREADS, MINB)
score_const_kernel(DeviceState s, int b, int chunk, int last_np, int arrivals, int H, int h_offset, float thr) {
    constexpr int HPC = HPT * THREADS;
    __shared__ unsigned long long red[THREADS / 32];
    __shared__ int s_last;
    if (s.skip != nullptr && *s.skip != 0) return;
    const int tid = threadIdx.x;
    const int t = blockIdx.x;
    const float4* base = c_pts + blockIdx.y * chunk;
    const int np = (blockIdx.y == gridDim.y - 1) ? last_np : chunk;
    const float nthr = -thr;
    const ThrScale ts = make_thr_scale(thr);
    (void)ts;
    const float* Eb = s.Ecand + (size_t)b * 9 * s.h_stride;
    float e[HPT][9];
    unsigned int cnt[HPT];
#pragma unroll
    for (int j = 0; j < HPT; j++) {
        int h = t * HPC + j * THREADS + tid;
        bool valid = h < H;
#pragma unroll
        for (int k = 0; k < 9; k++) {
            float v = valid ? __ldg(Eb + (size_t)k * s.h_stride + h) : 0.0f;
            if (MODEL != 1 && k != 8) v *= thr_scale_factor(ts, k);
            e[j][k] = v;
        }
        cnt[j] = 0u;
    }
#pragma unroll 4
    for (int i = 0; i < np; i++) {
        const float4 p = base[i];
#pragma unroll
        for (int j = 0; j < HPT; j++) {
            float dd = model_d<MODEL>(e[j], p.x, p.y, p.z, p.w, nthr);
            cnt[j] += __float_as_uint(dd) >> 31;
        }
    }
    segment_epilogue<HPT, THREADS>(s, b, t, H, h_offset, cnt, arrivals == 1, 1, arrivals, red, &s_last);
}

static int const_splits(int tiles, int batch, long long slots, int min_chunk = 64) {
    int max_s = batch / min_chunk;
    if (max_s < 1) max_s = 1;
    if (max_s > 512) max_s = 512;
    int best_s = 1;
    double best_eff = -1.0;
    for (int sp = 1; sp <= max_s; sp++) {
        double waves = (double)tiles * sp / (double)slots;
        double eff = waves / ceil(waves);
        if (eff > best_eff + 0.02) { best_eff = eff; best_s = sp; }
        if (eff > 0.985 && waves >= 2.0) break;
    }
    return best_s;
}

constexpr int CONST_HPT = 8, CONST_THREADS = 128, CONST_MINB = 4;

struct ConstBankGuard {
    std::mutex mu;
    cudaEvent_t last_use[64] = {};
};
static ConstBankGuard g_const;

template <int MODEL>
static void launch_score_const(const DeviceState& s, const ScorePlan& plan, int H, int h_offset, float thr, cudaStream_t st) {
    int dev = 0;
    cudaGetDevice(&dev);
    dev &= 63;
    std::lock_guard<std::mutex> lock(g_const.mu);
    if (!g_const.last_use[dev]) cudaEventCreateWithFlags(&g_const.last_use[dev], cudaEventDisableTiming);
    const int batches = (s.n + CONST_PTS - 1) / CONST_PTS;
    const int per = ((s.n + batches - 1) / batches + 15) / 16 * 16;
    int arrivals = 0;
    for (int off = 0; off < s.n; off += per) {
        const int cnt = s.n - off < per ? s.n - off : per;
        const int splits = const_splits(plan.tiles, cnt, plan.ctas);
        const int chunk = (cnt + splits - 1) / splits;
        arrivals += (cnt + chunk - 1) / chunk;
    }
    for (int b = 0; b < s.B; b++)
        for (int off = 0; off < s.n; off += per) {
            const int cnt = s.n - off < per ? s.n - off : per;
            const int splits = const_splits(plan.tiles, cnt, plan.ctas);
            const int chunk = (cnt + splits - 1) / splits;
            const int real_splits = (cnt + chunk - 1) / chunk;
            const int last_np = cnt - (real_splits - 1) * chunk;
            cudaStreamWaitEvent(st, g_const.last_use[dev], 0);
            cudaMemcpyToSymbolAsync(c_pts, s.corr_s + (size_t)b * s.n_stride + off, (size_t)cnt * sizeof(float4), 0,
                                    cudaMemcpyDeviceToDevice, st);
            score_const_kernel<CONST_HPT, CONST_THREADS, CONST_MINB, MODEL>
                <<<dim3(plan.tiles, real_splits), CONST_THREADS, 0, st>>>(s, b, chunk, last_np, arrivals, H, h_offset, thr);
            cudaEventRecord(g_const.last_use[dev], st);
        }
}

#ifndef SFMB200_V4_MINB
#define SFMB200_V4_MINB 1
#endif
#ifndef SFMB200_V8_MINB
#define SFMB200_V8_MINB 2
#endif
struct ScoreVariant { int hpt; int packed; int threads; int minb; };
static const ScoreVariant kVariants[] = {
    {2, 0, 256, 1}, {4, 1, 256, 1}, {4, 0, 256, 1}, {8, 0, 256, 2}, {8, 1, 256, SFMB200_V4_MINB},
    {4, 0, 128, 1}, {4, 1, 128, 1}, {8, 0, 128, 4}, {8, 1, 128, SFMB200_V8_MINB}, {2, 0, 128, 1},
    {CONST_HPT, 0, CONST_THREADS, CONST_MINB},
    {8, 1, 128, 3},
};
constexpr int kConstVariant = 10;
constexpr int kNumVariants = sizeof(kVariants) / sizeof(kVariants[0]);

template <int HPT, bool PACKED, int THREADS, int MINB>
static void launch_one(const DeviceState& s, int ctas, int H, int h_offset, int T, long long units, int n_units, float thr,
                       cudaStream_t st) {
    launch_dep(score_kernel<HPT, PACKED, THREADS, MINB, 0>, dim3(ctas), dim3(THREADS), 0, st, s, H, h_offset, T, units, n_units, thr);
}
template <int HPT, bool PACKED, int THREADS, int MINB>
static int occupancy_one() {
    int n = 0;
    cudaOccupancyMaxActiveBlocksPerMultiprocessor(&n, score_kernel<HPT, PACKED, THREADS, MINB, 0>, THREADS, 0);
    return n > 0 ? n : 1;
}
#define SFM_FOR_VARIANT(v, CALL)                     \
    switch (v) {                                     \
        case 0: CALL(2, false, 256, 1); break;       \
        case 1: CALL(4, true, 256, 1); break;        \
        case 2: CALL(4, false, 256, 1); break;       \
        case 3: CALL(8, false, 256, 2); break;       \
        case 4: CALL(8, true, 256, SFMB200_V4_MINB); break;        \
        case 5: CALL(4, false, 128, 1); break;       \
        case 6: CALL(4, true, 128, 1); break;        \
        case 7: CALL(8, false, 128, 4); break;       \
        case 8: CALL(8, true, 128, SFMB200_V8_MINB); break;        \
        case 11: CALL(8, true, 128, 3); break;       \
        default: CALL(2, false, 128, 1); break;      \
    }

static int variant_occupancy(int v) {
    static int cache[kNumVariants] = {0};
    if (cache[v] == 0 && v == kConstVariant) {
        int n = 0;
        cudaOccupancyMaxActiveBlocksPerMultiprocessor(&n, score_const_kernel<CONST_HPT, CONST_THREADS, CONST_MINB, 0>, CONST_THREADS, 0);
        cache[v] = n > 0 ? n : 1;
    }
    if (cache[v] == 0) {
#define SFM_OCC(h, p, t, m) cache[v] = occupancy_one<h, p, t, m>()
        SFM_FOR_VARIANT(v, SFM_OCC)
#undef SFM_OCC
    }
    return cache[v];
}

int score_num_variants() { return kNumVariants; }

ScorePlan make_score_plan(int B, int n, int H, int variant_override, int sms) {
    ScorePlan p;
    if (variant_override >= 0 && variant_override < kNumVariants) {
        p.variant = variant_override;
    } else {
        const double W = (double)B * (double)n * (double)H;
        if (H >= 1536) p.variant = W >= 1.2e8 ? 4 : 6;
        else if (H >= 768) p.variant = W >= 2e8 ? 1 : (W >= 3e7 ? 6 : 9);
        else p.variant = W >= 3e7 ? 6 : 9;
    }
    const ScoreVariant& v = kVariants[p.variant];
    p.hyp_per_cta = v.hpt * v.threads;
    p.tiles = (H + p.hyp_per_cta - 1) / p.hyp_per_cta;
    if (p.tiles < 1) p.tiles = 1;
    if (sms < 1) sms = 148;
    p.n_units = (n + SCORE_GRAIN - 1) / SCORE_GRAIN;
    p.total_units = (long long)B * p.tiles * p.n_units;
    long long ctas = (long long)sms * variant_occupancy(p.variant);
    if (p.variant != kConstVariant && ctas > p.total_units) ctas = p.total_units;
    if (ctas < 1) ctas = 1;
    p.ctas = (int)ctas;
    return p;
}

ScorePlan make_score_plan_homography(int B, int n, int H, int sms) {
#ifdef SFMB200_HOMOG_PLAN_BY_H
    return make_score_plan(B, n, H, H >= 1536 ? 4 : (H >= 384 ? 6 : 9), sms);
#else
    const double W = (double)B * (double)n * (double)H;
    return make_score_plan(B, n, H, H >= 1536 ? (W >= 1.2e8 ? 4 : 6) : (W >= 3e7 ? 6 : 9), sms);
#endif
}
template <int MODEL>
static void launch_score_model(const DeviceState& s, ScorePlan& plan, int H, int h_offset, float thr, cudaStream_t st) {
    const int v = plan.variant;
    if (v == kConstVariant) {
        launch_score_const<MODEL>(s, plan, H, h_offset, thr, st);
        return;
    }
    const bool big = kVariants[v].hpt * kVariants[v].threads >= 2048, mid = kVariants[v].hpt * kVariants[v].threads >= 512;
    if (big) {
        score_kernel<8, true, 256, 1, MODEL><<<plan.ctas, 256, 0, st>>>(s, H, h_offset, plan.tiles, plan.total_units, plan.n_units, thr);
    } else if (mid) {
        score_kernel<4, true, 128, 1, MODEL><<<plan.ctas, 128, 0, st>>>(s, H, h_offset, plan.tiles, plan.total_units, plan.n_units, thr);
    } else {
        score_kernel<2, false, 128, 1, MODEL><<<plan.ctas, 128, 0, st>>>(s, H, h_offset, plan.tiles, plan.total_units, plan.n_units, thr);
    }
}
void launch_score_homography(const DeviceState& s, ScorePlan& plan, int H, int h_offset, float thr2, cudaStream_t st) {
    launch_score_model<1>(s, plan, H, h_offset, thr2, st);
}
void launch_score_symmetric(const DeviceState& s, ScorePlan& plan, int H, int h_offset, float thr, cudaStream_t st) {
    launch_score_model<2>(s, plan, H, h_offset, thr, st);
}

void launch_score(const DeviceState& s, const ScorePlan& plan, int H, int h_offset, float thr, cudaStream_t st) {
    if (plan.variant == kConstVariant) {
        launch_score_const<0>(s, plan, H, h_offset, thr, st);
        return;
    }
#define SFM_LAUNCH(h, p, t, m) launch_one<h, p, t, m>(s, plan.ctas, H, h_offset, plan.tiles, plan.total_units, plan.n_units, thr, st)
    SFM_FOR_VARIANT(plan.variant, SFM_LAUNCH)
#undef SFM_LAUNCH
}

__global__ void select_kernel(DeviceState s, int h_offset) {
    const int b = blockIdx.x * blockDim.x + threadIdx.x;
    if (b >= s.B) return;
    unsigned long long packed = s.best[b];
    unsigned int hg = 0xFFFFFFFFu - (unsigned int)(packed & 0xFFFFFFFFull);
    int local = (int)hg - h_offset;
    s.best_idx[b] = (int)hg;
    s.best_count[b] = (int)(packed >> 32);
    const float* Eb = s.Ecand + (size_t)b * 9 * s.h_stride;
#pragma unroll
    for (int k = 0; k < 9; k++)
        s.E[(size_t)b * 9 + k] = (local >= 0 && local < s.h_stride) ? Eb[(size_t)k * s.h_stride + local] : 0.0f;
}

void launch_select(const DeviceState& s, int h_offset, cudaStream_t st) {
    select_kernel<<<(s.B + 127) / 128, 128, 0, st>>>(s, h_offset);
}

constexpr int PROBE_THREADS = 256;
constexpr int PROBE_CHAINS = 16;
constexpr int PROBE_INNER = 64;

template <int MODE>
__global__ void __launch_bounds__(PROBE_THREADS) fma_probe_kernel(int iters, float* sink, float a0, float b0) {
    if constexpr (MODE == 0) {
        float acc[PROBE_CHAINS];
        float a = a0 + threadIdx.x * 1e-9f, b = b0;
#pragma unroll
        for (int i = 0; i < PROBE_CHAINS; i++) acc[i] = (float)i;
        for (int it = 0; it < iters; it++) {
#pragma unroll
            for (int r = 0; r < PROBE_INNER; r++)
#pragma unroll
                for (int i = 0; i < PROBE_CHAINS; i++) acc[i] = fmaf(acc[i], a, b);
        }
        float t = 0.0f;
#pragma unroll
        for (int i = 0; i < PROBE_CHAINS; i++) t += acc[i];
        if (t == 123.456f) sink[0] = t;
    } else {
        float2 acc[PROBE_CHAINS];
        float2 a = make_float2(a0 + threadIdx.x * 1e-9f, a0), b = make_float2(b0, b0 * 0.5f);
#pragma unroll
        for (int i = 0; i < PROBE_CHAINS; i++) acc[i] = make_float2((float)i, (float)-i);
        for (int it = 0; it < iters; it++) {
#pragma unroll
            for (int r = 0; r < PROBE_INNER; r++)
#pragma unroll
                for (int i = 0; i < PROBE_CHAINS; i++) {
                    if constexpr (MODE == 1) acc[i] = __ffma2_rn(acc[i], a, b);
                    else if constexpr (MODE == 2) acc[i] = __fmul2_rn(acc[i], a);
                    else if constexpr (MODE == 3) acc[i] = __fadd2_rn(acc[i], b);
                    else acc[i] = __ffma2_rn(acc[i], a, make_float2(-acc[(i + 1) % PROBE_CHAINS].x, -acc[(i + 1) % PROBE_CHAINS].y));
                }
        }
        float t = 0.0f;
#pragma unroll
        for (int i = 0; i < PROBE_CHAINS; i++) t += acc[i].x + acc[i].y;
        if (t == 123.456f) sink[0] = t;
    }
}

double launch_fma_probe(int mode, int iters, cudaStream_t st, float* d_sink) {
    const int ctas = 148 * 8;
    if (mode == 0)
        fma_probe_kernel<0><<<ctas, PROBE_THREADS, 0, st>>>(iters, d_sink, 0.999f, 0.001f);
    else if (mode == 1)
        fma_probe_kernel<1><<<ctas, PROBE_THREADS, 0, st>>>(iters, d_sink, 0.999f, 0.001f);
    else if (mode == 2)
        fma_probe_kernel<2><<<ctas, PROBE_THREADS, 0, st>>>(iters, d_sink, 0.999f, 0.001f);
    else if (mode == 3)
        fma_probe_kernel<3><<<ctas, PROBE_THREADS, 0, st>>>(iters, d_sink, 0.999f, 0.001f);
    else
        fma_probe_kernel<4><<<ctas, PROBE_THREADS, 0, st>>>(iters, d_sink, 0.999f, 0.001f);
    double per_thread = (double)iters * PROBE_INNER * PROBE_CHAINS * (mode == 0 ? 1.0 : 2.0);
    return per_thread * PROBE_THREADS * ctas;
}

}
```

### cuda-sfm_b200/image_pair.py

```python
from __future__ import annotations

import ctypes as C

import numpy as np

from .binding import Lib, SfmError, load_library

OPT_COMPAT, OPT_SCORE_VARIANT, OPT_TRI_INLIERS_ONLY = 1, 2, 3


def _torch():
    import torch

    return torch


def _dptr(t, dtype: str | None = None, min_elems: int = 0) -> C.c_void_p:
    if t is None:
        return C.c_void_p(0)
    if isinstance(t, int):
        return C.c_void_p(t)
    if not (t.is_cuda and t.is_contiguous()):
        raise ValueError("expected a contiguous CUDA tensor")
    if dtype is not None and str(t.dtype) != "torch." + dtype:
        raise TypeError(f"expected a {dtype} tensor, got {t.dtype}")
    if t.numel() < min_elems:
        raise ValueError(f"tensor too small: {t.numel()} elements, need {min_elems}")
    return C.c_void_p(t.data_ptr())


def _hptr(a: np.ndarray, dtype=None, shape: tuple | None = None) -> C.c_void_p:
    if not isinstance(a, np.ndarray) or not a.flags["C_CONTIGUOUS"]:
        raise ValueError("expected a C-contiguous numpy array")
    if dtype is not None and a.dtype != np.dtype(dtype):
        raise TypeError(f"expected a {np.dtype(dtype)} array, got {a.dtype}")
    if shape is not None and tuple(a.shape) != tuple(shape):
        raise ValueError(f"expected shape {tuple(shape)}, got {tuple(a.shape)}")
    return C.c_void_p(a.ctypes.data)


class BatchedPairs:

    def __init__(self, K, Kinv, pairs: int, max_points: int, max_hypotheses: int, lib: Lib | None = None):
        self.lib = lib or load_library()
        self.K = np.ascontiguousarray(K, dtype=np.float32).reshape(9)
        self.Kinv = np.ascontiguousarray(Kinv, dtype=np.float32).reshape(9)
        self.pairs, self.max_points, self.max_hypotheses = pairs, max_points, max_hypotheses
        self.n = 0
        self.H = 0
        h = C.c_void_p()
        fp = C.POINTER(C.c_float)
        self.lib.call("sfmb200_create", self.K.ctypes.data_as(fp), self.Kinv.ctypes.data_as(fp), pairs, max_points,
                      max_hypotheses, C.byref(h))
        self._h = h
        self.use_torch_stream()

    def close(self):
        if getattr(self, "_h", None):
            self.lib.call("sfmb200_destroy", self._h)
            self._h = None

    def __del__(self):
        try:
            self.close()
        except Exception:
            pass

    def set_option(self, option: int, value: int):
        self.lib.call("sfmb200_set_option", self._h, option, value)

    def use_torch_stream(self, stream=None):
        torch = _torch()
        stream = stream or torch.cuda.current_stream()
        self.lib.call("sfmb200_set_stream", self._h, C.c_void_p(stream.cuda_stream))

    def synchronize(self):
        self.lib.call("sfmb200_synchronize", self._h)

    def set_points_sift(self, d_sift, n: int):
        self.lib.call("sfmb200_set_points_sift", self._h, _dptr(d_sift), n)
        self.n = n

    def set_points_sift_filtered(self, d_sift, n: int, min_score: float, max_ambiguity: float, d_kept_index=None) -> int:
        kept = C.c_int32(0)
        try:
            self.lib.call("sfmb200_set_points_sift_filtered", self._h, _dptr(d_sift), n, C.c_float(min_score),
                          C.c_float(max_ambiguity), _dptr(d_kept_index), C.byref(kept))
        finally:
            self.n = kept.value
        return kept.value

    def set_points_xy(self, d_px, n: int | None = None):
        n = n if n is not None else d_px.shape[-2]
        self.lib.call("sfmb200_set_points_xy", self._h, _dptr(d_px, "float32", self.pairs * n * 4), n)
        self.n = n

    def set_points_xy_host(self, h_px: np.ndarray):
        h_px = np.ascontiguousarray(h_px, dtype=np.float32)
        n = h_px.shape[-2]
        self.lib.call("sfmb200_set_points_xy_host", self._h, _hptr(h_px), n)
        self.synchronize()
        self.n = n

    def set_points_normalised(self, d_x, n: int | None = None):
        n = n if n is not None else d_x.shape[-2]
        self.lib.call("sfmb200_set_points_normalised", self._h, _dptr(d_x, "float32", self.pairs * n * 4), n)
        self.n = n

    def estimate_e(self, H: int, seed: int = 0, thr: float = 1e-6, d_idx=None, H_total: int | None = None, h_begin: int = 0):
        idx = _dptr(d_idx, "int32", self.pairs * (H_total or H) * 8)
        if H_total is None:
            self.lib.call("sfmb200_estimate_e", self._h, idx, H, C.c_uint64(seed), C.c_float(thr))
        else:
            self.lib.call("sfmb200_estimate_e_slice", self._h, idx, H_total, h_begin, H, C.c_uint64(seed), C.c_float(thr))
        self.H = H

    def estimate_e_adaptive(self, H_max: int, seed: int = 0, thr: float = 1e-6, confidence: float = 0.99,
                            first_round: int = 4096, growth: int = 4, d_idx=None) -> int:
        used = C.c_int32(0)
        self.lib.call("sfmb200_estimate_e_adaptive", self._h, _dptr(d_idx), H_max, first_round, growth, C.c_uint64(seed),
                      C.c_float(thr), C.c_float(confidence), C.byref(used))
        self.H = used.value
        return used.value

    def best_buffer(self):
        torch = _torch()
        p = C.c_void_p()
        self.lib.call("sfmb200_best_buffer", self._h, C.byref(p))
        return _tensor_from_ptr(p.value, (self.pairs,), torch.int64)

    def adopt_best(self, H_total: int, seed: int = 0, d_idx=None):
        self.lib.call("sfmb200_adopt_best", self._h, _dptr(d_idx), H_total, C.c_uint64(seed))

    def find_homography(self, loops: int, seed: int = 0, thresh: float = 5.0):
        Hm = np.empty((self.pairs, 3, 3), np.float32)
        cnt = np.empty(self.pairs, np.int32)
        self.lib.call("sfmb200_find_homography", self._h, loops, C.c_uint64(seed), C.c_float(thresh), _hptr(Hm), _hptr(cnt))
        self.H = loops
        return Hm, cnt

    def refine_e(self, iterations: int = 4) -> np.ndarray:
        self.lib.call("sfmb200_refine_e", self._h, iterations)
        out = np.empty(self.pairs, np.int32)
        self.lib.call("sfmb200_get_refit_iterations", self._h, _hptr(out))
        return out

    BA_STATS = ("active", "cost_entry", "cost", "accepted", "lambda", "gauge_scale", "inliers", "committed")

    def bundle_adjust(self, outer_rounds: int = 4, iterations: int = 40) -> np.ndarray:
        st = np.empty((self.pairs, 8), np.float32)
        self.lib.call("sfmb200_bundle_adjust", self._h, outer_rounds, iterations, _hptr(st))
        return st

    def chain_views(self, want_cloud: bool = True):
        torch = _torch()
        cams = np.empty((self.pairs + 1, 3, 4), np.float32)
        scales = np.empty(self.pairs, np.float32)
        used = np.empty(self.pairs, np.int32)
        cloud = torch.empty((4, self.n), dtype=torch.float32, device="cuda") if want_cloud else None
        count = torch.empty(self.n, dtype=torch.int32, device="cuda") if want_cloud else None
        self.lib.call("sfmb200_chain_views", self._h, _dptr(cloud), _dptr(count), _hptr(cams), _hptr(scales), _hptr(used))
        return dict(cameras=cams, scales=scales, used=used, cloud=cloud, count=count)

    GBA_STATS = ("cost_entry", "cost", "accepted", "lambda", "gauge_scale", "iterations", "spare0", "spare1")

    def bundle_adjust_global(self, chain: dict, iterations: int = 30):
        if chain.get("cloud") is None or chain.get("count") is None:
            raise ValueError("bundle_adjust_global needs the cloud and count of chain_views(want_cloud=True)")
        cams = np.empty((self.pairs + 1, 3, 4), np.float32)
        st = np.empty(8, np.float32)
        self.lib.call("sfmb200_bundle_adjust_global", self._h, _dptr(chain["cloud"], "float32", 4 * self.n), _dptr(chain["count"], "int32", self.n),
                      iterations, _hptr(cams), _hptr(st))
        chain["cameras"] = cams
        return st

    def pose_candidates(self):
        self.lib.call("sfmb200_pose_candidates", self._h)

    def choose_pose(self):
        self.lib.call("sfmb200_choose_pose", self._h)

    def triangulate(self):
        self.lib.call("sfmb200_triangulate", self._h)

    def run_device(self, d_px, H: int, seed: int = 0, thr: float = 1e-6, n: int | None = None):
        n = n if n is not None else d_px.shape[-2]
        self.lib.call("sfmb200_run_device", self._h, _dptr(d_px, "float32", self.pairs * n * 4), n, H, C.c_uint64(seed), C.c_float(thr))
        self.n, self.H = n, H

    def _host_io(self, h_px: np.ndarray, want_points: bool, out: dict | None):
        if not (isinstance(h_px, np.ndarray) and h_px.dtype == np.float32 and h_px.flags["C_CONTIGUOUS"]):
            h_px = np.ascontiguousarray(h_px, dtype=np.float32)
        if h_px.shape[-1] != 4 or h_px.size % 4 or h_px.size // 4 % self.pairs:
            raise ValueError(f"h_px must be [pairs={self.pairs}][n][4], got {h_px.shape}")
        n = h_px.size // 4 // self.pairs
        B = self.pairs
        if out is None:
            out = {"E": np.empty((B, 9), np.float32), "P": np.empty((B, 16), np.float32), "pose_index": np.empty(B, np.int32),
                   "inliers": np.empty(B, np.int32), "points": np.empty((B, 4, n), np.float32) if want_points else None}
        pts = out.get("points")
        ptrs = (_hptr(out["E"], np.float32, (B, 9)), _hptr(out["P"], np.float32, (B, 16)), _hptr(out["pose_index"], np.int32, (B,)),
                _hptr(out["inliers"], np.int32, (B,)), _hptr(pts, np.float32, (B, 4, n)) if pts is not None else C.c_void_p(0))
        return h_px, n, out, ptrs

    def run_host(self, h_px: np.ndarray, H: int, seed: int = 0, thr: float = 1e-6, want_points: bool = True, out: dict | None = None):
        h_px, n, out, ptrs = self._host_io(h_px, want_points, out)
        self.lib.call("sfmb200_run_host", self._h, _hptr(h_px), n, H, C.c_uint64(seed), C.c_float(thr), *ptrs)
        self.n, self.H = n, H
        return out

    def prepare_run_host(self, h_px: np.ndarray, H: int, seed: int = 0, thr: float = 1e-6, out: dict | None = None):
        h_px, n, out, ptrs = self._host_io(h_px, True, out)
        args = (self._h, _hptr(h_px), n, H, C.c_uint64(seed), C.c_float(thr), *ptrs)
        fn = self.lib.raw("sfmb200_run_host")
        lib = self.lib
        self.n, self.H = n, H

        def call():
            rc = fn(*args)
            if rc != 0:
                raise SfmError(rc, lib.last_error())
        call.keepalive = (h_px, out)
        return call, out

    def get_E(self) -> np.ndarray:
        out = np.empty((self.pairs, 3, 3), np.float32)
        self.lib.call("sfmb200_get_E", self._h, _hptr(out))
        return out

    def set_E(self, E: np.ndarray):
        E = np.ascontiguousarray(E, dtype=np.float32).reshape(self.pairs, 9)
        self.lib.call("sfmb200_set_E", self._h, _hptr(E))

    def get_best(self):
        idx = np.empty(self.pairs, np.int32)
        cnt = np.empty(self.pairs, np.int32)
        self.lib.call("sfmb200_get_best", self._h, _hptr(idx), _hptr(cnt))
        return idx, cnt

    def get_poses(self) -> np.ndarray:
        out = np.empty((self.pairs, 4, 4, 4), np.float32)
        self.lib.call("sfmb200_get_poses", self._h, _hptr(out))
        return out

    def get_pose_index(self) -> np.ndarray:
        out = np.empty(self.pairs, np.int32)
        self.lib.call("sfmb200_get_pose_index", self._h, _hptr(out))
        return out

    def get_points_host(self, pair: int = 0) -> np.ndarray:
        out = np.empty((4, self.n), np.float32)
        self.lib.call("sfmb200_get_points_host", self._h, pair, _hptr(out))
        return out

    def get_points(self, pair: int = 0):
        torch = _torch()
        out = torch.empty((4, self.n), dtype=torch.float32, device="cuda")
        self.lib.call("sfmb200_get_points", self._h, pair, _dptr(out))
        self.synchronize()
        return out

    def get_inlier_counts(self, pair: int = 0):
        torch = _torch()
        out = torch.empty(self.H, dtype=torch.int32, device="cuda")
        self.lib.call("sfmb200_get_inlier_counts", self._h, pair, _dptr(out))
        self.synchronize()
        return out

    def get_E_candidates(self, pair: int = 0):
        torch = _torch()
        out = torch.empty((self.H, 9), dtype=torch.float32, device="cuda")
        self.lib.call("sfmb200_get_E_candidates", self._h, pair, _dptr(out))
        self.synchronize()
        return out

    def get_X(self, image: int, pair: int = 0):
        torch = _torch()
        out = torch.empty((3, self.n), dtype=torch.float32, device="cuda")
        self.lib.call("sfmb200_get_X", self._h, pair, image, _dptr(out))
        self.synchronize()
        return out

    def get_inlier_mask(self, pair: int = 0):
        torch = _torch()
        out = torch.empty(self.n, dtype=torch.uint8, device="cuda")
        self.lib.call("sfmb200_get_inlier_mask", self._h, pair, _dptr(out))
        self.synchronize()
        return out

    def copy_to_vbo(self, d_pos, d_col, pair: int = 0):
        self.lib.call("sfmb200_copy_to_vbo", self._h, pair, _dptr(d_pos, "float32", 4 * self.n), _dptr(d_col, "float32", 4 * self.n))

    def copy_to_vbo_coloured(self, d_pos, d_col, pair: int = 0, scale: float = 1.0, mode: int = 1, z_near: float = 0.0, z_far: float = 1.0):
        self.lib.call("sfmb200_copy_to_vbo_coloured", self._h, pair, _dptr(d_pos, "float32", 4 * self.n), _dptr(d_col, "float32", 4 * self.n),
                      C.c_float(scale), mode,
                      C.c_float(z_near), C.c_float(z_far))

    def score_plan(self) -> dict:
        out = (C.c_int32 * 4)()
        self.lib.call("sfmb200_score_plan", self._h, out)
        return {"variant": out[0], "tiles": out[1], "ctas": out[2], "hyp_per_cta": out[3]}

    STAGES = ("ingest", "hypgen", "score", "select", "pose_candidates", "choose_pose", "triangulate")

    def stage_times(self, max_sets: int = 256) -> np.ndarray:
        ms = np.zeros((max_sets, 7), np.float32)
        sets = C.c_int(0)
        self.lib.call("sfmb200_stage_times", self._h, max_sets, _hptr(ms), C.byref(sets))
        return ms[: sets.value]

    def launch_count(self) -> int:
        return int(self.lib.raw("sfmb200_launch_count")(self._h))


def _tensor_from_ptr(ptr: int, shape, dtype):
    torch = _torch()
    n = int(np.prod(shape))
    itemsize = torch.empty((), dtype=dtype).element_size()

    class _Holder:
        __cuda_array_interface__ = {
            "shape": (n * itemsize,), "typestr": "|u1", "data": (ptr, False), "version": 3, "strides": None,
        }

    raw = torch.as_tensor(_Holder(), device="cuda")
    return raw.view(dtype).view(*shape)


class ImagePair(BatchedPairs):

    def __init__(self, k, k_inv, image_count: int, num_points: int, max_hypotheses: int | None = None, lib: Lib | None = None):
        if image_count != 2:
            raise ValueError("Image_pair handles exactly two images (like the reference)")
        self.image_count, self.num_points = image_count, num_points
        super().__init__(k, k_inv, 1, num_points, max_hypotheses or max(num_points // 8, 1), lib)

    def fillXU(self, data, n: int | None = None, min_score: float | None = None, max_ambiguity: float | None = None):
        if min_score is None and max_ambiguity is None:
            self.set_points_sift(data, n or self.num_points)
            return self.n
        return self.set_points_sift_filtered(data, n or self.num_points, min_score if min_score is not None else -np.inf,
                                             max_ambiguity if max_ambiguity is not None else np.inf)

    def estimateE(self, H: int | None = None, seed: int = 0, thr: float = 1e-6, d_idx=None):
        if H is None and d_idx is None:
            self.set_option(10, 1)
            try:
                self.estimate_e(max(self.n // 8, 1), seed, thr)
            finally:
                self.set_option(10, 0)
            return
        self.estimate_e(H or max(self.n // 8, 1), seed, thr, d_idx)

    def computePosecandidates(self):
        self.pose_candidates()

    def choosePose(self):
        self.choose_pose()

    def linear_triangulation(self):
        self.triangulate()

    def copyBoidsToVBO(self, vbodptr_positions, vbodptr_velocities):
        self.copy_to_vbo(vbodptr_positions, vbodptr_velocities)
```

### include/sfmb200.h

```cpp
#ifndef SFMB200_H
#define SFMB200_H

#include <stdint.h>

#ifdef __cplusplus
extern "C" {
#endif

typedef struct sfmb200_handle sfmb200_t;

typedef enum {
    SFMB200_OK = 0,
    SFMB200_ERR_ARG = -1,
    SFMB200_ERR_CUDA = -2,
    SFMB200_ERR_STATE = -3,
    SFMB200_ERR_NODEVICE = -4
} sfmb200_status;

typedef enum {
    SFMB200_OPT_COMPAT = 1,
    SFMB200_OPT_SCORE_VARIANT = 2,
    SFMB200_OPT_TRI_INLIERS_ONLY = 3,
    SFMB200_OPT_HYP_SOLVER = 5,
    SFMB200_OPT_PROFILE = 4,
    SFMB200_OPT_BA_PERSISTENT = 6,
    SFMB200_OPT_SMALL_PATH = 7,
    SFMB200_OPT_SMALL_PATH_EVALS = 8,
    SFMB200_OPT_BATCH_PIPELINE = 11,
    SFMB200_OPT_SAMPLER = 10,
    SFMB200_OPT_SCORE_METRIC = 9
} sfmb200_option;

const char* sfmb200_last_error(void);
int sfmb200_version(void);
const char* sfmb200_build_info(void);


int sfmb200_create(const float h_K[9], const float h_Kinv[9], int pairs, int max_points, int max_hypotheses,
                   sfmb200_t** out);
int sfmb200_destroy(sfmb200_t* h);
int sfmb200_set_option(sfmb200_t* h, int option, int value);
int sfmb200_set_stream(sfmb200_t* h, void* cuda_stream);
int sfmb200_synchronize(sfmb200_t* h);

int sfmb200_set_points_sift(sfmb200_t* h, const void* d_sift, int n);
int sfmb200_set_points_sift_filtered(sfmb200_t* h, const void* d_sift, int n, float min_score, float max_ambiguity,
                                     int32_t* d_kept_index, int32_t* h_kept);
int sfmb200_set_points_xy(sfmb200_t* h, const float* d_px, int n);
int sfmb200_set_points_xy_host(sfmb200_t* h, const float* h_px, int n);
int sfmb200_set_points_normalised(sfmb200_t* h, const float* d_x, int n);

int sfmb200_estimate_e(sfmb200_t* h, const int32_t* d_idx, int H, uint64_t seed, float thr);
int sfmb200_estimate_e_slice(sfmb200_t* h, const int32_t* d_idx, int H_total, int h_begin, int H, uint64_t seed,
                             float thr);
int sfmb200_estimate_e_adaptive(sfmb200_t* h, const int32_t* d_idx, int H_max, int first_round, int growth,
                                uint64_t seed, float thr, float confidence, int32_t* h_used);
int sfmb200_mg_handle_bytes(void);
int sfmb200_mg_init(sfmb200_t* h, int rank, int world, void* h_handle_out);
int sfmb200_mg_connect(sfmb200_t* h, const void* h_handles);
int sfmb200_estimate_e_mg(sfmb200_t* h, const int32_t* d_idx, int H_total, uint64_t seed, float thr);
int sfmb200_mg_status(sfmb200_t* h, int32_t* h_timeouts);
int sfmb200_mg_set_timeout_ms(sfmb200_t* h, int ms);
int sfmb200_mg_close(sfmb200_t* h);
int sfmb200_best_buffer(sfmb200_t* h, uint64_t** d_best);
int sfmb200_adopt_best(sfmb200_t* h, const int32_t* d_idx, int H_total, uint64_t seed);

int sfmb200_find_homography(sfmb200_t* h, int loops, uint64_t seed, float thresh, float* h_H, int32_t* h_matches);

int sfmb200_refine_e(sfmb200_t* h, int iterations);

int sfmb200_bundle_adjust(sfmb200_t* h, int outer_rounds, int iterations, float* h_stats);
int sfmb200_chain_views(sfmb200_t* h, float* d_cloud, int32_t* d_count, float* h_cameras, float* h_scales, int32_t* h_used);
int sfmb200_bundle_adjust_global(sfmb200_t* h, float* d_cloud, const int32_t* d_count, int iterations, float* h_cameras,
                                 float* h_stats);
int sfmb200_get_refit_iterations(sfmb200_t* h, int32_t* h_accepted );

int sfmb200_pose_candidates(sfmb200_t* h);
int sfmb200_choose_pose(sfmb200_t* h);
int sfmb200_triangulate(sfmb200_t* h);
int sfmb200_run_host(sfmb200_t* h, const float* h_px, int n, int H, uint64_t seed, float thr, float* h_E, float* h_P,
                     int32_t* h_pose_index, int32_t* h_inliers, float* h_points);
int sfmb200_run_device(sfmb200_t* h, const float* d_px, int n, int H, uint64_t seed, float thr);

int sfmb200_copy_to_vbo(sfmb200_t* h, int pair, float* d_pos, float* d_col);
int sfmb200_copy_to_vbo_coloured(sfmb200_t* h, int pair, float* d_pos, float* d_col, float scale, int mode, float z_near,
                                 float z_far);

int sfmb200_get_E(sfmb200_t* h, float* h_E );
int sfmb200_set_E(sfmb200_t* h, const float* h_E );
int sfmb200_get_best(sfmb200_t* h, int32_t* h_index, int32_t* h_count );
int sfmb200_get_poses(sfmb200_t* h, float* h_P );
int sfmb200_get_pose_index(sfmb200_t* h, int32_t* h_ind );
int sfmb200_get_points(sfmb200_t* h, int pair, float* d_points );
int sfmb200_get_points_host(sfmb200_t* h, int pair, float* h_points );
int sfmb200_get_inlier_counts(sfmb200_t* h, int pair, int32_t* d_counts );
int sfmb200_get_E_candidates(sfmb200_t* h, int pair, float* d_E );
int sfmb200_get_X(sfmb200_t* h, int pair, int image, float* d_X );
int sfmb200_get_inlier_mask(sfmb200_t* h, int pair, uint8_t* d_mask );
int sfmb200_device_views(sfmb200_t* h, float** d_E, float** d_P, int32_t** d_pose_index, float** d_points,
                         int* point_stride);
int sfmb200_score_plan(sfmb200_t* h, int32_t out[4]);
int64_t sfmb200_launch_count(sfmb200_t* h);
int sfmb200_stage_times(sfmb200_t* h, int max_sets, float* h_ms, int* sets);

int sfmb200_fma_probe(int mode, int iters, double* fmas, float* ms);

int sfmb200_small_path_debug(int64_t* d_stamps);

void sfmb200_host_svd3(const float a[9], float u[9], float s[9], float v[9]);
void sfmb200_host_svd3_reference_orientation(const float a[9], float u[9], float s[9], float v[9]);
void sfmb200_host_solve_hypothesis(const float pts[32], float E[9]);
void sfmb200_host_solve_hypothesis_projector(const float pts[32], float E[9]);
void sfmb200_host_null4(const float A[16], float x[4]);
int sfmb200_host_null4_fast(const float A[16], float x[4]);
int sfmb200_host_dlt_null(const float A[16], float x[4]);
void sfmb200_host_dlt_null_power4(const float A[16], float x[4]);
int sfmb200_host_inv4(const float m[16], float out[16]);
void sfmb200_host_sample_indices(uint64_t seed, uint64_t h, int n, int32_t idx[8]);
void sfmb200_host_sample_indices_disjoint(uint64_t seed, uint64_t h, int n, int32_t idx[8]);

#ifdef __cplusplus
}
#endif
#endif
```

Measured before the change: 1624 billion.

## Prune RANSAC hypotheses with a bounded lead-sweep cooperative scoring pass

Adds a pruned essential-matrix scoring mode, on by default, for large problems. It scores every hypothesis on a leading block of points, derives a bound from the current leader's count, and evaluates only surviving hypotheses on the remaining points. The whole pass runs in one cooperative kernel with grid-wide syncs. The aim is to skip correspondence evaluations for hypotheses that cannot win. The per-hypothesis counts left partial by pruning are recomputed lazily by a full counts kernel when a caller asks for counts or replaces the points, and a stats API reports how many evaluations were actually done. The exchange is extra grid syncs, more buffers, a fallback if the cooperative launch fails, and a deferred full rescore for callers that read counts.

```diff
diff --git a/cuda-sfm_b200/binding.py b/cuda-sfm_b200/binding.py
--- a/cuda-sfm_b200/binding.py
+++ b/cuda-sfm_b200/binding.py
@@ -73,6 +73,7 @@
     "sfmb200_get_inlier_mask": (C.c_int, [_vp, C.c_int, _vp]),
     "sfmb200_device_views": (C.c_int, [_vp, C.POINTER(_vp), C.POINTER(_vp), C.POINTER(_vp), C.POINTER(_vp), C.POINTER(C.c_int)]),
     "sfmb200_score_plan": (C.c_int, [_vp, _i]),
+    "sfmb200_score_stats": (C.c_int, [_vp, _vp, _vp]),
     "sfmb200_launch_count": (C.c_int64, [_vp]),
     "sfmb200_stage_times": (C.c_int, [_vp, C.c_int, _vp, C.POINTER(C.c_int)]),
     "sfmb200_fma_probe": (C.c_int, [C.c_int, C.c_int, C.POINTER(C.c_double), C.POINTER(C.c_float)]),
diff --git a/cuda-sfm_b200/csrc/api.cu b/cuda-sfm_b200/csrc/api.cu
--- a/cuda-sfm_b200/csrc/api.cu
+++ b/cuda-sfm_b200/csrc/api.cu
@@ -64,11 +64,16 @@
     int small_path;
     long long small_evals;
     int model;
+    int score_prune;
     int H;
     int h_begin;
     float thr;
     bool have_points, have_E, have_candidates, have_pose;
     ScorePlan plan;
+    bool pruned;
+    bool counts_partial;
+    int prune_tiles;
+    int prune_p0;
     int64_t launches;
     int* filter_scratch;
     float* pack_header;
@@ -116,6 +121,8 @@
     if (scope_.err != cudaSuccess) return fail(SFMB200_ERR_CUDA, "cannot make the handle's device current: %s", cudaGetErrorString(scope_.err))
 
 extern "C" {
+
+static int complete_counts(sfmb200_handle* h);
 
 const char* sfmb200_last_error(void) { return g_err; }
 int sfmb200_version(void) { return 100; }
@@ -153,6 +160,10 @@
     size_t o_ec = carve(B * 9 * (size_t)s.h_stride * sizeof(float));
     size_t o_cnt = carve(B * (size_t)s.h_stride * sizeof(int));
     size_t o_td = carve(B * (size_t)s.tiles_max * sizeof(int));
+    size_t o_win = carve(B * (size_t)s.tiles_max * sizeof(int));
+    size_t o_surv = carve(B * (size_t)s.h_stride * sizeof(int));
+    size_t o_pr = carve(B * 4 * sizeof(int));
+    size_t o_pc = carve(4 * sizeof(int));
     size_t o_best = carve(B * sizeof(unsigned long long));
     size_t o_E = carve(B * 9 * sizeof(float));
     size_t o_bi = carve(B * sizeof(int));
@@ -185,6 +196,10 @@
     s.Ecand = (float*)(base + o_ec);
     s.counts = (int*)(base + o_cnt);
     s.tile_done = (int*)(base + o_td);
+    s.winners = (int*)(base + o_win);
+    s.surv = (int*)(base + o_surv);
+    s.prune = (int*)(base + o_pr);
+    s.prune_ctl = (int*)(base + o_pc);
     s.best = (unsigned long long*)(base + o_best);
     s.E = (float*)(base + o_E);
     s.best_idx = (int*)(base + o_bi);
@@ -218,6 +233,7 @@
     h->compat = 1;
     h->hyp_solver = 1;
     h->score_variant = -1;
+    h->score_prune = 1;
     h->tri_inliers_only = 0;
     h->pipeline_chunks = -1;
     h->small_path = -1;
@@ -276,6 +292,10 @@
         case SFMB200_OPT_SAMPLER:
             if (value < 0 || value > 1) return fail(SFMB200_ERR_ARG, "sampler must be 0 (independent subsets) or 1 (disjoint permutation)%s");
             h->s.sampler = value;
+            break;
+        case SFMB200_OPT_SCORE_PRUNE:
+            if (value < 0 || value > 1) return fail(SFMB200_ERR_ARG, "score pruning must be 0 (evaluate everything) or 1 (prune)%s");
+            h->score_prune = value;
             break;
         case SFMB200_OPT_SCORE_METRIC:
             if (value < 0 || value > 1) return fail(SFMB200_ERR_ARG, "score metric must be 0 (Sampson error) or 1 (symmetric epipolar distance)%s");
@@ -336,6 +356,7 @@
     int rc = check_n(h, d_sift, n);
     if (rc) return rc;
     if (h->s.B != 1) return fail(SFMB200_ERR_ARG, "SiftPoint ingest needs pairs == 1%s");
+    if ((rc = complete_counts(h))) return rc;
     h->s.n = n;
     launch_ingest_sift(h->s, d_sift, n, h->stream);
     CKL();
@@ -350,6 +371,7 @@
     int rc = check_n(h, d_sift, n);
     if (rc) return rc;
     if (h->s.B != 1) return fail(SFMB200_ERR_ARG, "SiftPoint ingest needs pairs == 1%s");
+    if ((rc = complete_counts(h))) return rc;
     h->have_points = false;
     launch_ingest_sift_filtered(h->s, d_sift, n, min_score, max_ambiguity, h->filter_scratch, d_kept_index, h->stream);
     CKL();
@@ -381,6 +403,8 @@
 }
 int sfmb200_set_points_xy(sfmb200_t* h, const float* d_px, int n) {
     ENTER(h);
+    int rc = check_n(h, d_px, n);
+    if (rc || (rc = complete_counts(h))) return rc;
     return ingest_xy(h, d_px, n, 0.0f);
 }
 static int ensure_staging(sfmb200_handle* h, bool in, bool out) {
@@ -404,12 +428,14 @@
 }
 int sfmb200_set_points_xy_host(sfmb200_t* h, const float* h_px, int n) {
     ENTER(h);
+    int rc = check_n(h, h_px, n);
+    if (rc || (rc = complete_counts(h))) return rc;
     return ingest_xy_host(h, h_px, n, 0.0f);
 }
 int sfmb200_set_points_normalised(sfmb200_t* h, const float* d_x, int n) {
     ENTER(h);
     int rc = check_n(h, d_x, n);
-    if (rc) return rc;
+    if (rc || (rc = complete_counts(h))) return rc;
     h->s.n = n;
     launch_ingest_normalised(h->s, d_x, n, h->stream);
     CKL();
@@ -428,12 +454,32 @@
     return SFMB200_OK;
 }
 
-static void score_essential(sfmb200_handle* h, const DeviceState& s, int H, int h_offset, float thr) {
-    if (s.metric == 0) launch_score(s, h->plan, H, h_offset, thr, h->stream);
-    else launch_score_symmetric(s, h->plan, H, h_offset, thr, h->stream);
-}
 static ScorePlan plan_essential(const sfmb200_handle* h, int n, int H) {
     return h->s.metric == 0 ? make_score_plan(h->s.B, n, H, h->score_variant, h->sms) : make_score_plan_homography(h->s.B, n, H, h->sms);
+}
+static void score_essential(sfmb200_handle* h, const DeviceState& s, int H, int h_offset, float thr) {
+    if (s.metric == 0 && s.skip == nullptr && h->score_prune && !h->profile && score_prune_applies(h->plan, s.B, s.n, H)) {
+        h->prune_p0 = launch_score_pruned(s, h->plan, H, h_offset, thr, h->stream);
+        if (h->prune_p0 > 0) {
+            h->pruned = h->counts_partial = true;
+            h->prune_tiles = h->plan.tiles;
+        }
+    } else if (s.metric == 0) {
+        launch_score(s, h->plan, H, h_offset, thr, h->stream);
+    } else {
+        launch_score_symmetric(s, h->plan, H, h_offset, thr, h->stream);
+    }
+}
+static void begin_estimate(sfmb200_handle* h) { h->pruned = h->counts_partial = false; }
+static int complete_counts(sfmb200_handle* h) {
+    if (!h->counts_partial || !h->have_candidates) return SFMB200_OK;
+    h->counts_partial = false;
+    CK(cudaMemsetAsync(h->s.counts, 0, (size_t)h->s.B * h->s.h_stride * sizeof(int), h->stream));
+    const ScorePlan p = plan_essential(h, h->s.n, h->H);
+    launch_score_counts(h->s, p, h->H, h->h_begin, h->thr, h->stream);
+    CKL();
+    h->launches++;
+    return SFMB200_OK;
 }
 
 constexpr int SMALL_PATH_MAX_PAIRS = 4;
@@ -457,6 +503,7 @@
     if (!(thr > 0.0f)) return fail(SFMB200_ERR_ARG, "threshold must be positive%s");
     if (!d_idx && h->s.sampler == 1 && 8ll * H_total > (long long)h->s.n)
         return fail(SFMB200_ERR_ARG, "the disjoint-permutation sampler needs 8 * H_total <= n (the reference uses H = N / 8)%s");
+    begin_estimate(h);
     h->H = H;
     h->h_begin = h_begin;
     h->thr = thr;
@@ -502,6 +549,7 @@
     const float thresh_n = thresh / f;
     const float thr2 = thresh_n * thresh_n;
     if (int rc = ensure_scaled(h, 1.0f)) return rc;
+    begin_estimate(h);
     h->H = loops;
     h->h_begin = 0;
     h->thr = thr2;
@@ -568,6 +616,7 @@
     const double log1mp = log1p(-(double)confidence);
     if (int rc = ensure_scaled(h, make_thr_scale(thr).ik)) return rc;
     CK(cudaMemsetAsync(h->adapt, 0, 4 * sizeof(int), h->stream));
+    begin_estimate(h);
     DeviceState s = h->s;
     s.skip = h->adapt;
     long long lo = 0, hi = first_round;
@@ -942,6 +991,7 @@
     if (!h->have_points) return fail(SFMB200_ERR_STATE, "run before set_points%s");
     if (H < 1 || H > h->s.h_max) return fail(SFMB200_ERR_ARG, "H out of range / above max_hypotheses%s");
     if (!(thr > 0.0f)) return fail(SFMB200_ERR_ARG, "threshold must be positive%s");
+    begin_estimate(h);
     h->H = H;
     h->h_begin = 0;
     h->thr = thr;
@@ -1013,6 +1063,7 @@
     cudaError_t e = launch_small_path(h->s, d_px, nullptr, (long long)H * 8, H, 0, seed, thr, h->compat, h->tri_inliers_only,
                                       SMALL_INGEST | SMALL_ESTIMATE | SMALL_POSE | SMALL_TRI, h->stream);
     if (e != cudaSuccess) return fail(SFMB200_ERR_CUDA, "fused small-problem launch: %s", cudaGetErrorString(e));
+    begin_estimate(h);
     h->H = H;
     h->h_begin = 0;
     h->thr = thr;
@@ -1212,6 +1263,7 @@
     int rc = check_pair(h, pair, d_counts);
     if (rc) return rc;
     if (!h->have_candidates) return fail(SFMB200_ERR_STATE, "no estimate yet%s");
+    if ((rc = complete_counts(h))) return rc;
     CK(cudaMemcpyAsync(d_counts, h->s.counts + (size_t)pair * h->s.h_stride, (size_t)h->H * sizeof(int),
                        cudaMemcpyDeviceToDevice, h->stream));
     return SFMB200_OK;
@@ -1268,6 +1320,40 @@
     return SFMB200_OK;
 }
 int64_t sfmb200_launch_count(sfmb200_t* h) { return h ? h->launches : 0; }
+
+int sfmb200_score_stats(sfmb200_t* h, int64_t* h_evals, int32_t* h_stats) {
+    ENTER(h);
+    if (!h || !h_evals || !h_stats) return fail(SFMB200_ERR_ARG, "null argument%s");
+    if (!h->have_candidates) return fail(SFMB200_ERR_STATE, "no estimate with per-hypothesis scoring yet%s");
+    const int B = h->s.B;
+    const long long H = h->H, n = h->s.n, T = h->prune_tiles, P0 = h->prune_p0;
+    if (!h->pruned) {
+        for (int b = 0; b < B; b++) {
+            h_evals[b] = H * n;
+            h_stats[3 * b] = -1;
+            h_stats[3 * b + 1] = (int32_t)n;
+            h_stats[3 * b + 2] = (int32_t)H;
+        }
+        return SFMB200_OK;
+    }
+    int* tmp = new (std::nothrow) int[(size_t)B * 4];
+    if (!tmp) return fail(SFMB200_ERR_ARG, "out of host memory%s");
+    cudaError_t e = cudaMemcpyAsync(tmp, h->s.prune, (size_t)B * 4 * sizeof(int), cudaMemcpyDeviceToHost, h->stream);
+    if (e == cudaSuccess) e = cudaStreamSynchronize(h->stream);
+    if (e != cudaSuccess) {
+        delete[] tmp;
+        return fail(SFMB200_ERR_CUDA, "score_stats: %s", cudaGetErrorString(e));
+    }
+    for (int b = 0; b < B; b++) {
+        const long long L = tmp[4 * b], S = tmp[4 * b + 1], P1 = tmp[4 * b + 2];
+        h_evals[b] = H * P1 + T * (n - P0) + S * (n - P1);
+        h_stats[3 * b] = (int32_t)L;
+        h_stats[3 * b + 1] = (int32_t)P1;
+        h_stats[3 * b + 2] = (int32_t)S;
+    }
+    delete[] tmp;
+    return SFMB200_OK;
+}
 
 int sfmb200_stage_times(sfmb200_t* h, int max_sets, float* ms, int* sets) {
     ENTER(h);
diff --git a/cuda-sfm_b200/csrc/internal.cuh b/cuda-sfm_b200/csrc/internal.cuh
--- a/cuda-sfm_b200/csrc/internal.cuh
+++ b/cuda-sfm_b200/csrc/internal.cuh
@@ -39,6 +39,10 @@
     float* Ecand;
     int* counts;
     int* tile_done;
+    int* winners;
+    int* surv;
+    int* prune;
+    int* prune_ctl;
     unsigned long long* best;
     float* E;
     int* best_idx;
@@ -63,6 +67,9 @@
     v.Ecand += b * 9 * s.h_stride;
     v.counts += b * s.h_stride;
     v.tile_done += b * s.tiles_max;
+    v.winners += b * s.tiles_max;
+    v.surv += b * s.h_stride;
+    v.prune += b * 4;
     v.best += b;
     v.E += b * 9;
     v.best_idx += b;
@@ -155,6 +162,10 @@
 ScorePlan make_score_plan(int B, int n, int H, int variant_override, int sms);
 int score_num_variants();
 void launch_score(const DeviceState& s, const ScorePlan& plan, int H, int h_offset, float thr, cudaStream_t st);
+constexpr int PRUNE_P0 = SCORE_CHUNK;
+bool score_prune_applies(const ScorePlan& plan, int B, int n, int H);
+int launch_score_pruned(const DeviceState& s, const ScorePlan& plan, int H, int h_offset, float thr, cudaStream_t st);
+void launch_score_counts(const DeviceState& s, const ScorePlan& plan, int H, int h_offset, float thr, cudaStream_t st);
 void launch_score_homography(const DeviceState& s, ScorePlan& plan, int H, int h_offset, float thr2, cudaStream_t st);
 void launch_score_symmetric(const DeviceState& s, ScorePlan& plan, int H, int h_offset, float thr, cudaStream_t st);
 ScorePlan make_score_plan_homography(int B, int n, int H, int sms);
diff --git a/cuda-sfm_b200/csrc/score.cu b/cuda-sfm_b200/csrc/score.cu
--- a/cuda-sfm_b200/csrc/score.cu
+++ b/cuda-sfm_b200/csrc/score.cu
@@ -4,12 +4,16 @@
 
 #include "internal.cuh"
 #include "sampson.cuh"
+
+#include <cooperative_groups.h>
 
 #ifndef SFMB200_SCORE_UNROLL
 #define SFMB200_SCORE_UNROLL 2
 #endif
 
 namespace sfmb200 {
+
+namespace cg = cooperative_groups;
 
 constexpr int kScoreUnroll = SFMB200_SCORE_UNROLL;
 
@@ -53,13 +57,14 @@
 
 struct ChunkWalk {
     long long u, end;
-    int n_units, n, T;
+    int n_units, T;
+    int p_begin, p_end;
     int b, t, p0, cnt;
     int seg_p0, seg_pts;
     int left;
     bool seg_first, seg_last;
-    __device__ __forceinline__ void init(long long u0, long long u1, int n_units_, int n_, int T_) {
-        u = u0; end = u1; n_units = n_units_; n = n_; T = T_;
+    __device__ __forceinline__ void init(long long u0, long long u1, int n_units_, int p_begin_, int p_end_, int T_) {
+        u = u0; end = u1; n_units = n_units_; p_begin = p_begin_; p_end = p_end_; T = T_;
         left = 0; cnt = 0; p0 = 0;
     }
     __device__ __forceinline__ bool next() {
@@ -71,9 +76,9 @@
             if (seg_units > n_units - pu) seg_units = n_units - pu;
             b = (int)(bt / T);
             t = (int)(bt - (long long)b * T);
-            seg_p0 = pu * SCORE_GRAIN;
-            int p1 = (pu + (int)seg_units) * SCORE_GRAIN;
-            if (p1 > n) p1 = n;
+            seg_p0 = p_begin + pu * SCORE_GRAIN;
+            int p1 = p_begin + (pu + (int)seg_units) * SCORE_GRAIN;
+            if (p1 > p_end) p1 = p_end;
             seg_pts = p1 - seg_p0;
             left = seg_pts;
             u += seg_units;
@@ -90,66 +95,173 @@
     }
 };
 
+enum ScorePhase { PH_FULL = 0, PH_LEAD = 1, PH_SWEEP = 2, PH_COUNTS = 3, PH_PRUNED = 4 };
+constexpr int PRUNE_RHO_INV = 10;
+
+struct ScorePass {
+    int phase;
+    int p_begin, p_end;
+    int T;
+};
+
+__device__ __forceinline__ int prune_cut(int n, int L, int p0) {
+    long long p1 = ((long long)(n - L) * PRUNE_RHO_INV + PRUNE_RHO_INV - 2) / (PRUNE_RHO_INV - 1);
+    p1 = (p1 + SCORE_GRAIN - 1) / SCORE_GRAIN * SCORE_GRAIN;
+    if (p1 < p0 + SCORE_GRAIN) p1 = p0 + SCORE_GRAIN;
+    return p1 > n ? n : (int)p1;
+}
+
+template <int MODEL>
+__device__ void list_score(const DeviceState& s, const int* list, int stride, const int* cnt4, int cnt_fixed, int maxcnt, int pb,
+                           int pe, float thr) {
+    const long long R = pe - pb;
+    const long long total = (long long)s.B * maxcnt * R;
+    if (R <= 0 || total <= 0) return;
+    const long long nt = (long long)gridDim.x * blockDim.x;
+    const long long g = (long long)blockIdx.x * blockDim.x + threadIdx.x;
+    long long w = total * g / nt;
+    const long long w1 = total * (g + 1) / nt;
+    const ThrScale ts = make_thr_scale(thr);
+    const float nthr = -thr;
+    (void)ts;
+    while (w < w1) {
+        const long long item = w / R;
+        const int b = (int)(item / maxcnt), i = (int)(item - (long long)b * maxcnt);
+        const long long end = (item + 1) * R < w1 ? (item + 1) * R : w1;
+        const int cnt_b = cnt4 ? __ldcg(cnt4 + 4 * b) : cnt_fixed;
+        if (i < cnt_b) {
+            const int h = __ldcg(list + (size_t)b * stride + i);
+            const float* Eb = s.Ecand + (size_t)b * 9 * s.h_stride + h;
+            float e[9];
+#pragma unroll
+            for (int q = 0; q < 9; q++) {
+                float v = __ldg(Eb + (size_t)q * s.h_stride);
+                if (MODEL != 1 && q != 8) v *= thr_scale_factor(ts, q);
+                e[q] = v;
+            }
+            const float4* pts = s.corr_s + (size_t)b * s.n_stride + pb;
+            unsigned int c = 0u;
+            for (long long x = w - item * R; x < end - item * R; x++) {
+                const float4 p = pts[x];
+                c += __float_as_uint(model_d<MODEL>(e, p.x, p.y, p.z, p.w, nthr)) >> 31;
+            }
+            if (c != 0u) atomicAdd(&s.counts[(size_t)b * s.h_stride + h], (int)c);
+        }
+        w = end;
+    }
+}
+__device__ void list_keys(const DeviceState& s, const int* list, int stride, const int* cnt4, int cnt_fixed, int maxcnt, int h_offset,
+                          bool bound) {
+    const long long items = (long long)s.B * maxcnt;
+    for (long long it = (long long)blockIdx.x * blockDim.x + threadIdx.x; it < items; it += (long long)gridDim.x * blockDim.x) {
+        const int b = (int)(it / maxcnt), i = (int)(it - (long long)b * maxcnt);
+        if (i >= (cnt4 ? __ldcg(cnt4 + 4 * b) : cnt_fixed)) continue;
+        const int h = __ldcg(list + (size_t)b * stride + i);
+        const int c = __ldcg(&s.counts[(size_t)b * s.h_stride + h]);
+        atomicMax(&s.best[b], ((unsigned long long)(unsigned int)c << 32) | (unsigned long long)(0xFFFFFFFFu - (unsigned)(h_offset + h)));
+        if (bound) atomicMax(&s.prune[4 * b], c);
+    }
+}
+
 template <int HPT, int THREADS>
-__device__ __forceinline__ void segment_epilogue(const DeviceState& s, int b, int t, int H, int h_offset,
+__device__ __forceinline__ void segment_epilogue(const DeviceState& s, const ScorePass& ps, int b, int t, int H, int h_offset,
                                                  const unsigned int* cnt, bool full, int inc, int total,
                                                  unsigned long long* red, int* s_last) {
     constexpr int HPC = HPT * THREADS;
     const int tid = threadIdx.x;
+    const int phase = ps.phase;
+    const bool add = ps.p_begin > 0;
+    const int lead = phase == PH_SWEEP ? __ldcg(&s.winners[(size_t)b * s.tiles_max + t]) : -1;
     int* counts = s.counts + (size_t)b * s.h_stride;
-    unsigned long long key = 0ull;
+    int hyp[HPT];
+    unsigned int tot[HPT];
     bool do_argmax;
+#pragma unroll
+    for (int j = 0; j < HPT; j++) {
+        const int pos = t * HPC + j * THREADS + tid;
+        hyp[j] = pos < H ? pos : -1;
+    }
     if (full) {
 #pragma unroll
         for (int j = 0; j < HPT; j++) {
-            int h = t * HPC + j * THREADS + tid;
-            if (h < H) {
-                counts[h] = (int)cnt[j];
-                unsigned long long kk = ((unsigned long long)cnt[j] << 32) |
-                                        (unsigned long long)(0xFFFFFFFFu - (unsigned)(h_offset + h));
-                key = kk > key ? kk : key;
+            const int h = hyp[j];
+            if (h >= 0 && h != lead) {
+                tot[j] = (add ? (unsigned int)counts[h] : 0u) + cnt[j];
+                counts[h] = (int)tot[j];
+            } else if (h >= 0) {
+                tot[j] = (unsigned int)counts[h];
             }
         }
         do_argmax = true;
     } else {
 #pragma unroll
         for (int j = 0; j < HPT; j++) {
-            int h = t * HPC + j * THREADS + tid;
-            if (h < H && cnt[j] != 0u) atomicAdd(&counts[h], (int)cnt[j]);
+            const int h = hyp[j];
+            if (h >= 0 && h != lead && cnt[j] != 0u) atomicAdd(&counts[h], (int)cnt[j]);
         }
         __threadfence();
         __syncthreads();
         if (tid == 0) {
-            int before = atomicAdd(&s.tile_done[(size_t)b * s.tiles_max + t], inc);
+            int* ticket = &s.tile_done[(size_t)b * s.tiles_max + t];
+            int before = atomicAdd(ticket, inc);
             *s_last = (before + inc == total);
+            if (before + inc == total) *ticket = 0;
         }
         __syncthreads();
         do_argmax = *s_last != 0;
         if (do_argmax) {
             __threadfence();
 #pragma unroll
-            for (int j = 0; j < HPT; j++) {
-                int h = t * HPC + j * THREADS + tid;
-                if (h < H) {
-                    unsigned int total = (unsigned int)__ldcg(&counts[h]);
-                    unsigned long long kk = ((unsigned long long)total << 32) |
-                                            (unsigned long long)(0xFFFFFFFFu - (unsigned)(h_offset + h));
-                    key = kk > key ? kk : key;
-                }
-            }
-        }
-    }
-    if (do_argmax) {
-        key = warp_max_u64(key);
-        if ((tid & 31) == 0) red[tid >> 5] = key;
-        __syncthreads();
-        if (tid < 32) {
-            unsigned long long v = tid < THREADS / 32 ? red[tid] : 0ull;
-            v = warp_max_u64(v);
-            if (tid == 0 && v != 0ull) atomicMax(&s.best[b], v);
-        }
-        __syncthreads();
-    }
+            for (int j = 0; j < HPT; j++)
+                if (hyp[j] >= 0) tot[j] = (unsigned int)__ldcg(&counts[hyp[j]]);
+        }
+    }
+    if (!do_argmax || phase == PH_COUNTS) return;
+    if (phase == PH_SWEEP && tid == 0) s.prune[4 * b + 2] = ps.p_end;
+    if (phase == PH_SWEEP && ps.p_end < s.n) {
+        const int P1 = ps.p_end;
+        const unsigned int L = (unsigned int)__ldcg(&s.prune[4 * b]);
+        const unsigned int rest = (unsigned int)(s.n - P1);
+        const int lane = tid & 31;
+#pragma unroll
+        for (int j = 0; j < HPT; j++) {
+            const bool keep = hyp[j] >= 0 && hyp[j] != lead && tot[j] + rest >= L;
+            const unsigned int m = __ballot_sync(0xFFFFFFFFu, keep);
+            if (m == 0u) continue;
+            int base = 0;
+            if (lane == 0) {
+                base = atomicAdd(&s.prune[4 * b + 1], __popc(m));
+                atomicMax(&s.prune_ctl[1], base + __popc(m));
+            }
+            base = __shfl_sync(0xFFFFFFFFu, base, 0);
+            if (keep) s.surv[(size_t)b * s.h_stride + base + __popc(m & ((1u << lane) - 1u))] = hyp[j];
+        }
+        return;
+    }
+    unsigned long long key = 0ull;
+#pragma unroll
+    for (int j = 0; j < HPT; j++) {
+        if (hyp[j] >= 0) {
+            unsigned long long kk = ((unsigned long long)tot[j] << 32) |
+                                    (unsigned long long)(0xFFFFFFFFu - (unsigned)(h_offset + hyp[j]));
+            key = kk > key ? kk : key;
+        }
+    }
+    key = warp_max_u64(key);
+    if ((tid & 31) == 0) red[tid >> 5] = key;
+    __syncthreads();
+    if (tid < 32) {
+        unsigned long long v = tid < THREADS / 32 ? red[tid] : 0ull;
+        v = warp_max_u64(v);
+        if (tid == 0 && v != 0ull) {
+            if (phase == PH_LEAD) {
+                s.winners[(size_t)b * s.tiles_max + t] = (int)(0xFFFFFFFFu - (unsigned int)(v & 0xFFFFFFFFull)) - h_offset;
+            } else {
+                atomicMax(&s.best[b], v);
+            }
+        }
+    }
+    __syncthreads();
 }
 
 struct ChunkDesc {
@@ -160,7 +272,7 @@
 
 template <int HPT, bool PACKED, int THREADS, int MINB, int MODEL>
 __global__ void __launch_bounds__(THREADS, MINB)
-score_kernel(DeviceState s, int H, int h_offset, int T, long long total_units, int n_units, float thr) {
+score_kernel(DeviceState s, int H, int h_offset, int T, long long total_units, int n_units, float thr, int phase) {
     constexpr int HPC = HPT * THREADS;
     __shared__ __align__(128) float4 buf[2][SCORE_CHUNK];
     __shared__ __align__(8) uint64_t full[2];
@@ -168,20 +280,13 @@
     __shared__ ChunkWalk walk;
     __shared__ unsigned long long red[THREADS / 32];
     __shared__ int s_last;
+    __shared__ ScorePass pass;
 
     pdl_wait();
-    pdl_trigger();
+    if (phase != PH_PRUNED) pdl_trigger();
     if (s.skip != nullptr && *s.skip != 0) return;
     const int tid = threadIdx.x;
-    if (tid == 0) {
-        mbar_init(&full[0], 1);
-        mbar_init(&full[1], 1);
-        asm volatile("fence.mbarrier_init.release.cluster;" ::: "memory");
-        ChunkWalk w;
-        w.init(total_units * blockIdx.x / gridDim.x, total_units * (blockIdx.x + 1) / gridDim.x, n_units, s.n, T);
-        walk = w;
-    }
-    __syncthreads();
+    __shared__ int s_cut;
 
     auto produce = [&](int stage) {
         ChunkWalk w = walk;
@@ -200,7 +305,6 @@
             mbar_expect_tx(&full[stage], 0);
         }
     };
-    if (tid == 0) produce(0);
 
     float e[PACKED ? 1 : HPT][9];
     float2 e2[PACKED ? HPT / 2 : 1][9];
@@ -210,60 +314,132 @@
     const ThrScale ts = make_thr_scale(thr);
     (void)e; (void)e2; (void)nthr2; (void)ts;
 
-    for (int k = 0;; k++) {
-        if (tid == 0) produce((k + 1) & 1);
-        mbar_wait(&full[k & 1], (k >> 1) & 1);
-        const ChunkDesc d = desc[k & 1];
-        if (d.cnt_flags == 0) break;
-        const int n_here = d.cnt_flags & 0x3FFFFFFF;
-        if (d.cnt_flags & (1 << 30)) {
-            const float* Eb = s.Ecand + (size_t)d.b * 9 * s.h_stride;
-#pragma unroll
-            for (int j = 0; j < HPT; j++) {
-                int h = d.t * HPC + j * THREADS + tid;
-                bool valid = h < H;
-#pragma unroll
-                for (int q = 0; q < 9; q++) {
-                    float v = valid ? __ldg(Eb + (size_t)q * s.h_stride + h) : 0.0f;
-                    if (MODEL != 1 && q != 8) v *= thr_scale_factor(ts, q);
-                    if constexpr (PACKED) {
-                        if (j & 1) e2[j / 2][q].y = v; else e2[j / 2][q].x = v;
-                    } else {
-                        e[j][q] = v;
+    const int p0 = phase == PH_PRUNED ? n_units * SCORE_GRAIN : 0;
+    const int walks = phase == PH_PRUNED ? 2 : 1;
+    for (int wi = 0; wi < walks; wi++) {
+        const int ph = phase == PH_PRUNED ? (wi == 0 ? PH_LEAD : PH_SWEEP) : phase;
+        if constexpr (MODEL == 0) {
+            if (ph == PH_SWEEP) {
+                cg::grid_group grid = cg::this_grid();
+                grid.sync();
+                list_score<MODEL>(s, s.winners, s.tiles_max, nullptr, T, T, p0, s.n, thr);
+                grid.sync();
+                list_keys(s, s.winners, s.tiles_max, nullptr, T, T, h_offset, true);
+                grid.sync();
+                if (tid == 0) s_cut = p0 + SCORE_GRAIN;
+                __syncthreads();
+                for (int b = tid; b < s.B; b += THREADS) atomicMax(&s_cut, prune_cut(s.n, __ldcg(&s.prune[4 * b]), p0));
+                __syncthreads();
+                if (tid == 0) {
+                    asm volatile("mbarrier.inval.shared::cta.b64 [%0];" ::"r"(smem_u32(&full[0])) : "memory");
+                    asm volatile("mbarrier.inval.shared::cta.b64 [%0];" ::"r"(smem_u32(&full[1])) : "memory");
+                }
+            }
+        }
+        if (tid == 0) {
+            mbar_init(&full[0], 1);
+            mbar_init(&full[1], 1);
+            asm volatile("fence.mbarrier_init.release.cluster;" ::: "memory");
+            ScorePass ps;
+            ps.phase = ph;
+            ps.p_begin = 0;
+            ps.p_end = s.n;
+            ps.T = T;
+            long long units = total_units;
+            int nu = n_units;
+            if (ph == PH_LEAD) {
+                ps.p_end = p0;
+                if (blockIdx.x == 0) s.prune_ctl[1] = 0;
+            } else if (ph == PH_SWEEP) {
+                ps.p_begin = p0;
+                const long long per = (long long)s.B * T;
+                const long long u = per * ((s_cut - p0 + SCORE_GRAIN - 1) / SCORE_GRAIN);
+                const long long fill = (u + gridDim.x - 1) / gridDim.x * gridDim.x / per;
+                const long long p1 = p0 + fill * SCORE_GRAIN;
+                ps.p_end = p1 < s.n ? (int)p1 : s.n;
+            }
+            if (ph == PH_LEAD || ph == PH_SWEEP) {
+                nu = (ps.p_end - ps.p_begin + SCORE_GRAIN - 1) / SCORE_GRAIN;
+                units = (long long)s.B * T * nu;
+            }
+            pass = ps;
+            ChunkWalk w;
+            w.init(units * blockIdx.x / gridDim.x, units * (blockIdx.x + 1) / gridDim.x, nu, ps.p_begin, ps.p_end, ps.T);
+            walk = w;
+        }
+        if (ph == PH_LEAD && blockIdx.x == 0)
+            for (int i = tid; i < 4 * s.B; i += THREADS) s.prune[i] = 0;
+        __syncthreads();
+        if (tid == 0) produce(0);
+
+        for (int k = 0;; k++) {
+            if (tid == 0) produce((k + 1) & 1);
+            mbar_wait(&full[k & 1], (k >> 1) & 1);
+            const ChunkDesc d = desc[k & 1];
+            if (d.cnt_flags == 0) break;
+            const int n_here = d.cnt_flags & 0x3FFFFFFF;
+            if (d.cnt_flags & (1 << 30)) {
+                const float* Eb = s.Ecand + (size_t)d.b * 9 * s.h_stride;
+#pragma unroll
+                for (int j = 0; j < HPT; j++) {
+                    const int h = d.t * HPC + j * THREADS + tid;
+                    const bool valid = h < H;
+#pragma unroll
+                    for (int q = 0; q < 9; q++) {
+                        float v = valid ? __ldg(Eb + (size_t)q * s.h_stride + h) : 0.0f;
+                        if (MODEL != 1 && q != 8) v *= thr_scale_factor(ts, q);
+                        if constexpr (PACKED) {
+                            if (j & 1) e2[j / 2][q].y = v; else e2[j / 2][q].x = v;
+                        } else {
+                            e[j][q] = v;
+                        }
+                    }
+                    cnt[j] = 0u;
+                }
+            }
+            const float4* pb = buf[k & 1];
+            if constexpr (PACKED) {
+#pragma unroll kScoreUnroll
+                for (int i = 0; i < n_here; i++) {
+                    const float4 p = pb[i];
+                    const float2 x1 = make_float2(p.x, p.x), y1 = make_float2(p.y, p.y);
+                    const float2 x2 = make_float2(p.z, p.z), y2 = make_float2(p.w, p.w);
+#pragma unroll
+                    for (int j = 0; j < HPT / 2; j++) {
+                        float2 dd = model_d2<MODEL>(e2[j], x1, y1, x2, y2, nthr2);
+                        cnt[2 * j] += __float_as_uint(dd.x) >> 31;
+                        cnt[2 * j + 1] += __float_as_uint(dd.y) >> 31;
                     }
                 }
-                cnt[j] = 0u;
-            }
-        }
-        const float4* pb = buf[k & 1];
-        if constexpr (PACKED) {
-#pragma unroll kScoreUnroll
-            for (int i = 0; i < n_here; i++) {
-                const float4 p = pb[i];
-                const float2 x1 = make_float2(p.x, p.x), y1 = make_float2(p.y, p.y);
-                const float2 x2 = make_float2(p.z, p.z), y2 = make_float2(p.w, p.w);
-#pragma unroll
-                for (int j = 0; j < HPT / 2; j++) {
-                    float2 dd = model_d2<MODEL>(e2[j], x1, y1, x2, y2, nthr2);
-                    cnt[2 * j] += __float_as_uint(dd.x) >> 31;
-                    cnt[2 * j + 1] += __float_as_uint(dd.y) >> 31;
+            } else {
+#pragma unroll 4
+                for (int i = 0; i < n_here; i++) {
+                    float4 p = pb[i];
+#pragma unroll
+                    for (int j = 0; j < HPT; j++) {
+                        float dd = model_d<MODEL>(e[j], p.x, p.y, p.z, p.w, nthr);
+                        cnt[j] += __float_as_uint(dd) >> 31;
+                    }
                 }
             }
-        } else {
-#pragma unroll 4
-            for (int i = 0; i < n_here; i++) {
-                float4 p = pb[i];
-#pragma unroll
-                for (int j = 0; j < HPT; j++) {
-                    float dd = model_d<MODEL>(e[j], p.x, p.y, p.z, p.w, nthr);
-                    cnt[j] += __float_as_uint(dd) >> 31;
-                }
-            }
-        }
-        __syncthreads();
-        if (d.cnt_flags >= 0) continue;
-
-        segment_epilogue<HPT, THREADS>(s, d.b, d.t, H, h_offset, cnt, d.seg_pts == s.n, d.seg_pts, s.n, red, &s_last);
+            __syncthreads();
+            if (d.cnt_flags >= 0) continue;
+
+            const int range = pass.p_end - pass.p_begin;
+            segment_epilogue<HPT, THREADS>(s, pass, d.b, d.t, H, h_offset, cnt, d.seg_pts == range, d.seg_pts, range, red, &s_last);
+        }
+    }
+    if constexpr (MODEL == 0) {
+        if (phase == PH_PRUNED) {
+            cg::grid_group grid = cg::this_grid();
+            grid.sync();
+            const int P1 = pass.p_end;
+            const int maxs = __ldcg(&s.prune_ctl[1]);
+            list_score<MODEL>(s, s.surv, s.h_stride, s.prune + 1, 0, maxs, P1, s.n, thr);
+            grid.sync();
+            pdl_trigger();
+            list_keys(s, s.surv, s.h_stride, s.prune + 1, 0, maxs, h_offset, false);
+        }
     }
 }
 
@@ -308,7 +484,8 @@
             cnt[j] += __float_as_uint(dd) >> 31;
         }
     }
-    segment_epilogue<HPT, THREADS>(s, b, t, H, h_offset, cnt, arrivals == 1, 1, arrivals, red, &s_last);
+    const ScorePass ps = {PH_FULL, 0, s.n, (int)gridDim.x};
+    segment_epilogue<HPT, THREADS>(s, ps, b, t, H, h_offset, cnt, arrivals == 1, 1, arrivals, red, &s_last);
 }
 
 static int const_splits(int tiles, int batch, long long slots, int min_chunk = 64) {
@@ -384,8 +561,9 @@
 
 template <int HPT, bool PACKED, int THREADS, int MINB>
 static void launch_one(const DeviceState& s, int ctas, int H, int h_offset, int T, long long units, int n_units, float thr,
-                       cudaStream_t st) {
-    launch_dep(score_kernel<HPT, PACKED, THREADS, MINB, 0>, dim3(ctas), dim3(THREADS), 0, st, s, H, h_offset, T, units, n_units, thr);
+                       cudaStream_t st, int phase = PH_FULL) {
+    launch_dep(score_kernel<HPT, PACKED, THREADS, MINB, 0>, dim3(ctas), dim3(THREADS), 0, st, s, H, h_offset, T, units, n_units, thr,
+               phase);
 }
 template <int HPT, bool PACKED, int THREADS, int MINB>
 static int occupancy_one() {
@@ -466,11 +644,11 @@
     }
     const bool big = kVariants[v].hpt * kVariants[v].threads >= 2048, mid = kVariants[v].hpt * kVariants[v].threads >= 512;
     if (big) {
-        score_kernel<8, true, 256, 1, MODEL><<<plan.ctas, 256, 0, st>>>(s, H, h_offset, plan.tiles, plan.total_units, plan.n_units, thr);
+        score_kernel<8, true, 256, 1, MODEL><<<plan.ctas, 256, 0, st>>>(s, H, h_offset, plan.tiles, plan.total_units, plan.n_units, thr, PH_FULL);
     } else if (mid) {
-        score_kernel<4, true, 128, 1, MODEL><<<plan.ctas, 128, 0, st>>>(s, H, h_offset, plan.tiles, plan.total_units, plan.n_units, thr);
+        score_kernel<4, true, 128, 1, MODEL><<<plan.ctas, 128, 0, st>>>(s, H, h_offset, plan.tiles, plan.total_units, plan.n_units, thr, PH_FULL);
     } else {
-        score_kernel<2, false, 128, 1, MODEL><<<plan.ctas, 128, 0, st>>>(s, H, h_offset, plan.tiles, plan.total_units, plan.n_units, thr);
+        score_kernel<2, false, 128, 1, MODEL><<<plan.ctas, 128, 0, st>>>(s, H, h_offset, plan.tiles, plan.total_units, plan.n_units, thr, PH_FULL);
     }
 }
 void launch_score_homography(const DeviceState& s, ScorePlan& plan, int H, int h_offset, float thr2, cudaStream_t st) {
@@ -486,6 +664,44 @@
         return;
     }
 #define SFM_LAUNCH(h, p, t, m) launch_one<h, p, t, m>(s, plan.ctas, H, h_offset, plan.tiles, plan.total_units, plan.n_units, thr, st)
+    SFM_FOR_VARIANT(plan.variant, SFM_LAUNCH)
+#undef SFM_LAUNCH
+}
+
+template <int HPT, bool PACKED, int THREADS, int MINB>
+static cudaError_t launch_pruned_one(DeviceState s, int ctas, int H, int h_offset, int T, int p0_grains, float thr, cudaStream_t st) {
+    long long units = 0;
+    int phase = PH_PRUNED;
+    void* args[] = {&s, &H, &h_offset, &T, &units, &p0_grains, &thr, &phase};
+    return cudaLaunchCooperativeKernel((const void*)score_kernel<HPT, PACKED, THREADS, MINB, 0>, dim3(ctas), dim3(THREADS), args, 0, st);
+}
+
+bool score_prune_applies(const ScorePlan& plan, int B, int n, int H) {
+    return plan.variant != kConstVariant && n >= 4 * PRUNE_P0 && H >= 16384 && (double)B * (double)n * (double)H >= 1e8;
+}
+
+int launch_score_pruned(const DeviceState& s, const ScorePlan& plan, int H, int h_offset, float thr, cudaStream_t st) {
+    const int T = plan.tiles;
+    const long long per = (long long)s.B * T;
+    long long g = PRUNE_P0 / SCORE_GRAIN;
+    g = (per * g + plan.ctas - 1) / plan.ctas * plan.ctas / per;
+    if (g * SCORE_GRAIN > s.n / 2) g = s.n / 2 / SCORE_GRAIN;
+    if (g < PRUNE_P0 / SCORE_GRAIN) g = PRUNE_P0 / SCORE_GRAIN;
+    cudaError_t e = cudaErrorInvalidValue;
+#define SFM_LAUNCH(h, p, t, m) e = launch_pruned_one<h, p, t, m>(s, plan.ctas, H, h_offset, T, (int)g, thr, st)
+    SFM_FOR_VARIANT(plan.variant, SFM_LAUNCH)
+#undef SFM_LAUNCH
+    if (e != cudaSuccess) {
+        cudaGetLastError();
+        launch_score(s, plan, H, h_offset, thr, st);
+        return 0;
+    }
+    return (int)g * SCORE_GRAIN;
+}
+
+void launch_score_counts(const DeviceState& s, const ScorePlan& plan, int H, int h_offset, float thr, cudaStream_t st) {
+#define SFM_LAUNCH(h, p, t, m) \
+    launch_one<h, p, t, m>(s, plan.ctas, H, h_offset, plan.tiles, plan.total_units, plan.n_units, thr, st, PH_COUNTS)
     SFM_FOR_VARIANT(plan.variant, SFM_LAUNCH)
 #undef SFM_LAUNCH
 }
diff --git a/cuda-sfm_b200/image_pair.py b/cuda-sfm_b200/image_pair.py
--- a/cuda-sfm_b200/image_pair.py
+++ b/cuda-sfm_b200/image_pair.py
@@ -7,6 +7,7 @@
 from .binding import Lib, SfmError, load_library
 
 OPT_COMPAT, OPT_SCORE_VARIANT, OPT_TRI_INLIERS_ONLY = 1, 2, 3
+OPT_SCORE_PRUNE = 12
 
 
 def _torch():
@@ -301,6 +302,12 @@
         self.lib.call("sfmb200_score_plan", self._h, out)
         return {"variant": out[0], "tiles": out[1], "ctas": out[2], "hyp_per_cta": out[3]}
 
+    def score_stats(self) -> dict:
+        evals = np.zeros(self.pairs, np.int64)
+        st = np.zeros((self.pairs, 3), np.int32)
+        self.lib.call("sfmb200_score_stats", self._h, _hptr(evals), _hptr(st))
+        return {"evals": evals, "L": st[:, 0].copy(), "P1": st[:, 1].copy(), "survivors": st[:, 2].copy()}
+
     STAGES = ("ingest", "hypgen", "score", "select", "pose_candidates", "choose_pose", "triangulate")
 
     def stage_times(self, max_sets: int = 256) -> np.ndarray:
diff --git a/include/sfmb200.h b/include/sfmb200.h
--- a/include/sfmb200.h
+++ b/include/sfmb200.h
@@ -28,6 +28,7 @@
     SFMB200_OPT_SMALL_PATH_EVALS = 8,
     SFMB200_OPT_BATCH_PIPELINE = 11,
     SFMB200_OPT_SAMPLER = 10,
+    SFMB200_OPT_SCORE_PRUNE = 12,
     SFMB200_OPT_SCORE_METRIC = 9
 } sfmb200_option;
 
@@ -100,6 +101,7 @@
 int sfmb200_device_views(sfmb200_t* h, float** d_E, float** d_P, int32_t** d_pose_index, float** d_points,
                          int* point_stride);
 int sfmb200_score_plan(sfmb200_t* h, int32_t out[4]);
+int sfmb200_score_stats(sfmb200_t* h, int64_t* h_evals, int32_t* h_stats);
 int64_t sfmb200_launch_count(sfmb200_t* h);
 int sfmb200_stage_times(sfmb200_t* h, int max_sets, float* h_ms, int* sets);
 
```

Result: faster. 2734 billion, median of 6 (+68.4%).
